# jonathanking/protein-transformer

Measured on AMD Instinct MI355X. Metric: train-step residues/sec (enc-only d512, drmsd loss), higher is better.
Workload: dtype f32 (GEMM and attention operands scaled by powers of two and split into 2 f16 terms [activation x weight products, weight-gradient products whose operands come with a uniform scale, attention with head size 64 / 32] or exactly into 3 bf16 terms [the other weight-gradient products; everything when to; 1 GPU; enc-only d_model=512 n_layers=6 n_head=8 d_ff=2048, -l drmsd, sgd lr 1e-4 wd 0.01 clip 1, dropout 0.1, 32 proteins x L=512 per GPU (BASELINE.json configs[3]); global_batch=32, seq_len=512, parallelism=dp1

## Files before the change

### include/ptamd.h

```cpp
#ifndef PTAMD_H
#define PTAMD_H

#include <stddef.h>
#include <stdint.h>

#ifdef __cplusplus
extern "C" {
#endif

#define PTAMD_OK 0
#define PTAMD_ERR_BAD_SHAPE (-1)
#define PTAMD_ERR_TOO_LONG (-2)
#define PTAMD_ERR_WORKSPACE (-3)
#define PTAMD_ERR_HIP (-4)
#define PTAMD_ERR_ALIGN (-5)

#define PTAMD_ST_BAD_RESIDUE 1
#define PTAMD_ST_TOO_SHORT 2
#define PTAMD_ST_BAD_THETA 4
#define PTAMD_ST_NONFINITE 8

#define PTAMD_PAD_ID 20
#define PTAMD_NUM_ANGLES 12
#define PTAMD_NUM_SLOTS 14
// ... 4 lines not shown

int ptamd_angles_fwd(const float *sincos, float *ang, int64_t n, void *stream);
int ptamd_angles_bwd(const float *sincos, const float *dang, float *dsincos, int64_t n, void *stream);

size_t ptamd_nerf_workspace_bytes(int B, int L);
int ptamd_nerf_place(const float *a, const float *b, const float *c, const float *l, const float *theta,
                     const float *chi, int64_t n, float *d, int32_t *status, void *stream);
int ptamd_pairwise_dist(const float *x, int n, int dim, float *out, void *stream);
int ptamd_nerf_fwd(const float *ang, const int64_t *seq, int B, int L, float *crd, int32_t *status,
                   void *stream);
int ptamd_nerf_bwd(const float *ang, const int64_t *seq, const float *crd, const float *dcrd, int B, int L,
                   float *dang, void *workspace, size_t workspace_bytes, void *stream);

size_t ptamd_drmsd_workspace_bytes(int B, int L);
int ptamd_drmsd_fwd_bwd(const float *pred_crd, const float *true_crd, const int64_t *seq, int B, int L,
                        float *stats, float *dcrd, void *workspace, size_t workspace_bytes, void *stream);
size_t ptamd_drmsd_workspace_bytes_budget(int B, int L, size_t partial_budget_bytes);
int ptamd_drmsd_fwd_bwd_budget(const float *pred_crd, const float *true_crd, const int64_t *seq, int B, int L,
                               float *stats, float *dcrd, void *workspace, size_t workspace_bytes,
                               size_t partial_budget_bytes, void *stream);

int ptamd_kabsch_rmsd(const float *pred_crd, const float *true_crd, const int64_t *seq, int B, int L, float *rmsd,
                      void *stream);

size_t ptamd_mse_angles_workspace_bytes(void);
int ptamd_mse_angles_fwd(const float *pred, const float *truth, int64_t T, float *out, void *workspace,
                         size_t workspace_bytes, void *stream);
int ptamd_mse_angles_bwd(const float *pred, const float *truth, int64_t T, const float *sums, float coef,
                         int accumulate, float *dpred, void *stream);

#define PTAMD_EPI_RELU 1
#define PTAMD_EPI_TANH 2
#define PTAMD_EPI_ACCUM 4
#define PTAMD_EPI_SLABS 16
#define PTAMD_EPI_GATE 8
typedef struct {
  int M, N, K;
  const float *A; int lda; int a_kmajor;
  const float *B; int ldb; int b_kmajor;
  float *C; int ldc;
  const float *bias;
  const float *residual; int ldr;
  int flags;
  float dropout_p; uint64_t seed; uint32_t stream_id;
  int split_k;
  void *workspace; size_t workspace_bytes;
  float *colsum;
  float gate_scale;
  int arith;
  int reserved_cus;
  const uint32_t *a_scale; int a_scale_stride;
  const uint32_t *b_scale; int b_scale_stride;
  const uint64_t *gate_mask;
} ptamd_gemm_args;
size_t ptamd_gate_mask_bytes(int M, int N);
size_t ptamd_gemm_workspace_bytes(int M, int N, int split_k);
int ptamd_gemm(const ptamd_gemm_args *args, void *stream);

#define PTAMD_GEMM_F32 0
#define PTAMD_GEMM_BF16X3 1
#define PTAMD_GEMM_BF16X3_FULL 2
#define PTAMD_GEMM_F16X2 3
#define PTAMD_GEMM_AUTO 4
int ptamd_gemm_products(const ptamd_gemm_args *args);
int ptamd_gemm_group(const ptamd_gemm_args *args, int n, void *stream);

size_t ptamd_hp_bytes(int rows, int K);
int ptamd_hp_padded_rows(int rows);
int ptamd_hp_split(const float *x, int ld, int rows, int K, int transposed, void *planes, float *scale, void *stream);
typedef struct {
  const float *x; int ld, rows, K;
  void *planes; float *scale;
} ptamd_hp_split_job;
int ptamd_hp_split_rows(const ptamd_hp_split_job *jobs_host, int njobs, void *stream);
int ptamd_hp_split_cols(const ptamd_hp_split_job *jobs_host, int njobs, void *stream);
typedef struct {
  int M, N, K;
  const void *A; const float *A_scale;
  const void *B; const float *B_scale;
  float *C; int ldc;
  const float *bias;
  const float *residual; int ldr;
  int flags;
  float dropout_p; uint64_t seed; uint32_t stream_id;
  int split_k;
  void *workspace; size_t workspace_bytes;
  float gate_scale;
  int reserved_cus;
  const uint64_t *gate_mask;
  uint64_t *gate_mask_out;
  void *kv_planes; float *kv_inv; int kv_col0, kv_heads;
} ptamd_gemm_hp_args;
size_t ptamd_gemm_hp_workspace_bytes(int M, int N, int split_k);
int ptamd_gemm_hp(const ptamd_gemm_hp_args *args, void *stream);

typedef struct {
  const float *w; int rows, cols, ld;
  uint32_t *row_scale; uint32_t *col_scale; float *stats;
  int rows_only;
} ptamd_wscale_job;
int ptamd_weight_scales(const ptamd_wscale_job *jobs_host, int njobs, void *stream);
typedef struct {
  const float *ln_gamma_stats; const float *ln_beta_stats;
  const float *w_stats; int w_stat_index;
  const float *bias_stats;
  float sqrt_d, post_scale;
  uint32_t *out_scale; float *out_value;
} ptamd_bound_job;
int ptamd_bound_scales(const ptamd_bound_job *jobs_host, int njobs, void *stream);
typedef struct { uint32_t *dst; int64_t n; uint32_t value; } ptamd_fill_job;
int ptamd_fill_u32(const ptamd_fill_job *jobs_host, int njobs, void *stream);

typedef struct {
  int64_t offset;
  int32_t rows, cols;
  int32_t stats_row0;
  int32_t stats_index;
  int32_t row_scale_index;
  int32_t col_scale_index;
  int32_t colmax_index;
  int32_t colsq_index;
  uint64_t row_planes;
  uint64_t col_planes;
  int32_t ld;
  int32_t rowmax_index;
} ptamd_wprep_seg;
typedef struct {
  int32_t ln_gamma_stats, ln_beta_stats, w_stats, w_stat_index, bias_stats;
  float sqrt_d, post_scale;
  int32_t out_scale, out_value;
} ptamd_wprep_bound;
typedef struct {
  const ptamd_wprep_seg *segs; int32_t nsegs;
  const int32_t *blocks_a; int32_t nblocks_a, nblocks_a_matrices;
  const int64_t *plain; int32_t nplain;
  const int32_t *blocks_b; int32_t nblocks_b;
  const ptamd_wprep_bound *bounds; int32_t nbounds;
  const int32_t *groups; int32_t ngroups;
  const int32_t *colnorm_segs;
  uint32_t *scales; float *values;
  uint32_t *colmax; int32_t ncolmax;
  void *colsq;
  float *stats; int32_t nstats;
  int64_t numel;
// ... 81 lines not shown
```

### protein_transformer_amd/_lib.py

```python
import ctypes as C
import os

import torch

_HERE = os.path.dirname(os.path.abspath(__file__))
_TAG = os.environ.get("PTAMD_LIB_TAG", "")
LIB_PATH = os.path.join(_HERE, "csrc", f"libptamd_{_TAG}.so" if _TAG else "libptamd.so")

OK = 0
ERRORS = {-1: "bad shape", -2: "sequence too long for the NeRF LDS staging", -3: "workspace missing or too small",
          -4: "HIP runtime error", -5: "pointer not 16-byte aligned"}
ST_BAD_RESIDUE, ST_TOO_SHORT, ST_BAD_THETA, ST_NONFINITE = 1, 2, 4, 8

_p, _i, _i64, _f, _sz, _u64, _u32 = C.c_void_p, C.c_int, C.c_int64, C.c_float, C.c_size_t, C.c_uint64, C.c_uint32


class GemmArgs(C.Structure):
    _fields_ = [("M", _i), ("N", _i), ("K", _i),
                ("A", _p), ("lda", _i), ("a_kmajor", _i),
                ("B", _p), ("ldb", _i), ("b_kmajor", _i),
                ("C", _p), ("ldc", _i),
                ("bias", _p),
                ("residual", _p), ("ldr", _i),
                ("flags", _i),
                ("dropout_p", _f), ("seed", _u64), ("stream_id", _u32),
                ("split_k", _i),
                ("workspace", _p), ("workspace_bytes", _sz),
                ("colsum", _p),
                ("gate_scale", _f),
                ("arith", _i),
                ("reserved_cus", _i),
                ("a_scale", _p), ("a_scale_stride", _i),
                ("b_scale", _p), ("b_scale_stride", _i),
                ("gate_mask", _p)]


class WScaleJob(C.Structure):
    _fields_ = [("w", _p), ("rows", _i), ("cols", _i), ("ld", _i), ("row_scale", _p), ("col_scale", _p), ("stats", _p),
                ("rows_only", _i)]


class BoundJob(C.Structure):
    _fields_ = [("ln_gamma_stats", _p), ("ln_beta_stats", _p), ("w_stats", _p), ("w_stat_index", _i), ("bias_stats", _p),
                ("sqrt_d", _f), ("post_scale", _f), ("out_scale", _p), ("out_value", _p)]


class LnReduceJob(C.Structure):
    _fields_ = [("partials", _p), ("D", _i), ("dgamma", _p), ("dbeta", _p)]


class FillJob(C.Structure):
    _fields_ = [("dst", _p), ("n", _i64), ("value", _u32)]


class HpSplitJob(C.Structure):
    _fields_ = [("x", _p), ("ld", _i), ("rows", _i), ("K", _i), ("planes", _p), ("scale", _p)]


class GemmHpArgs(C.Structure):
    _fields_ = [("M", _i), ("N", _i), ("K", _i),
                ("A", _p), ("A_scale", _p),
                ("B", _p), ("B_scale", _p),
                ("C", _p), ("ldc", _i),
                ("bias", _p),
                ("residual", _p), ("ldr", _i),
                ("flags", _i),
                ("dropout_p", _f), ("seed", _u64), ("stream_id", _u32),
                ("split_k", _i),
                ("workspace", _p), ("workspace_bytes", _sz),
                ("gate_scale", _f),
                ("reserved_cus", _i),
                ("gate_mask", _p), ("gate_mask_out", _p),
                ("kv_planes", _p), ("kv_inv", _p), ("kv_col0", _i), ("kv_heads", _i)]


class WprepSeg(C.Structure):
    _fields_ = [("offset", _i64), ("rows", C.c_int32), ("cols", C.c_int32), ("stats_row0", C.c_int32), ("stats_index", C.c_int32),
                ("row_scale_index", C.c_int32), ("col_scale_index", C.c_int32), ("colmax_index", C.c_int32),
                ("colsq_index", C.c_int32), ("row_planes", _u64), ("col_planes", _u64), ("ld", C.c_int32), ("rowmax_index", C.c_int32)]


class WprepBound(C.Structure):
    _fields_ = [("ln_gamma_stats", C.c_int32), ("ln_beta_stats", C.c_int32), ("w_stats", C.c_int32), ("w_stat_index", C.c_int32),
                ("bias_stats", C.c_int32), ("sqrt_d", _f), ("post_scale", _f), ("out_scale", C.c_int32), ("out_value", C.c_int32)]


class WprepPlan(C.Structure):
    _fields_ = [("segs", _p), ("nsegs", C.c_int32),
                ("blocks_a", _p), ("nblocks_a", C.c_int32), ("nblocks_a_matrices", C.c_int32),
                ("plain", _p), ("nplain", C.c_int32),
                ("blocks_b", _p), ("nblocks_b", C.c_int32),
                ("bounds", _p), ("nbounds", C.c_int32),
                ("groups", _p), ("ngroups", C.c_int32),
                ("colnorm_segs", _p),
                ("scales", _p), ("values", _p),
                ("colmax", _p), ("ncolmax", C.c_int32),
                ("colsq", _p),
                ("stats", _p), ("nstats", C.c_int32),
                ("numel", _i64), ("with_planes", C.c_int32)]


SIGNATURES = {
    "ptamd_version": (C.c_char_p, []),
    "ptamd_last_hip_error": (C.c_char_p, []),
    "ptamd_sidechain_atoms": (_i, [_i]),
    "ptamd_angles_fwd": (_i, [_p, _p, _i64, _p]),
    "ptamd_angles_bwd": (_i, [_p, _p, _p, _i64, _p]),
    "ptamd_nerf_workspace_bytes": (_sz, [_i, _i]),
    "ptamd_nerf_place": (_i, [_p, _p, _p, _p, _p, _p, _i64, _p, _p, _p]),
    "ptamd_pairwise_dist": (_i, [_p, _i, _i, _p, _p]),
    "ptamd_nerf_fwd": (_i, [_p, _p, _i, _i, _p, _p, _p]),
    "ptamd_nerf_bwd": (_i, [_p, _p, _p, _p, _i, _i, _p, _p, _sz, _p]),
    "ptamd_drmsd_workspace_bytes": (_sz, [_i, _i]),
    "ptamd_drmsd_fwd_bwd": (_i, [_p, _p, _p, _i, _i, _p, _p, _p, _sz, _p]),
    "ptamd_drmsd_workspace_bytes_budget": (_sz, [_i, _i, _sz]),
    "ptamd_drmsd_fwd_bwd_budget": (_i, [_p, _p, _p, _i, _i, _p, _p, _p, _sz, _sz, _p]),
    "ptamd_kabsch_rmsd": (_i, [_p, _p, _p, _i, _i, _p, _p]),
    "ptamd_mse_angles_workspace_bytes": (_sz, []),
    "ptamd_mse_angles_fwd": (_i, [_p, _p, _i64, _p, _p, _sz, _p]),
    "ptamd_mse_angles_bwd": (_i, [_p, _p, _i64, _p, _f, _i, _p, _p]),
    "ptamd_gemm_workspace_bytes": (_sz, [_i, _i, _i]),
    "ptamd_gate_mask_bytes": (_sz, [_i, _i]),
    "ptamd_gemm": (_i, [C.POINTER(GemmArgs), _p]),
    "ptamd_gemm_products": (_i, [C.POINTER(GemmArgs)]),
    "ptamd_gemm_group": (_i, [C.POINTER(GemmArgs), _i, _p]),
    "ptamd_hp_bytes": (_sz, [_i, _i]),
# ... 113 lines not shown
```

### protein_transformer_amd/csrc/gemm.hip

```cpp
#include <stdlib.h>

#include "gemm_common.h"

namespace ptgemm {
namespace {

template <bool KMAJOR, int BK>
__device__ __forceinline__ void store_stage(float *__restrict__ s, int tid, const float4 (&v)[BK / 8]) {
  constexpr int LPR = BK / 4, LD_R = BK + 4;
#pragma unroll
  for (int i = 0; i < BK / 8; ++i) {
    if (!KMAJOR) {
      const int row = tid / LPR + (NT / LPR) * i, k = 4 * (tid % LPR);
      *reinterpret_cast<float4 *>(s + row * LD_R + k) = v[i];
    } else {
      const int k = (tid >> 5) + 8 * i, row = 4 * (tid & 31);
      *reinterpret_cast<float4 *>(s + k * LD_C + row) = v[i];
    }
  }
}
template <bool KMAJOR, int BK>
__device__ __forceinline__ void read_frag(const float *__restrict__ s, int r, int lh, int m, float (&f)[4]) {
  constexpr int LD_R = BK + 4;
  if (!KMAJOR) {
// ... 329 lines not shown
  const size_t a_bytes = (size_t)(a->a_kmajor ? a->K : a->M) * a->lda * sizeof(float);
  const size_t b_bytes = (size_t)(a->b_kmajor ? a->K : a->N) * a->ldb * sizeof(float);
  if (mode == PTAMD_GEMM_F16X2 && a->K < 32) mode = PTAMD_GEMM_BF16X3;
  if (a->K < 16 || a_bytes >= ((size_t)1 << 32) || b_bytes >= ((size_t)1 << 32)) mode = PTAMD_GEMM_F32;
  return mode;
}
}

int ptamd_gemm_products(const ptamd_gemm_args *a) {
  if (!a || a->M <= 0 || a->N <= 0 || a->K <= 0 || !valid_arith(a->arith)) return PTAMD_ERR_BAD_SHAPE;
  const int mode = resolve_mode(a);
  return mode == PTAMD_GEMM_F32 ? 1 : mode == PTAMD_GEMM_F16X2 ? 3 : mode == PTAMD_GEMM_BF16X3_FULL ? 9 : 6;
}

namespace {
int build_params(const ptamd_gemm_args *a, GemmParams &p, int &splits, int &mode, float *&user_c) {
  if (!a || a->M <= 0 || a->N <= 0 || a->K <= 0 || !valid_arith(a->arith)) return PTAMD_ERR_BAD_SHAPE;
  if ((a->lda & 3) || (a->ldb & 3)) return PTAMD_ERR_BAD_SHAPE;
  if ((!a->a_kmajor || !a->b_kmajor) && (a->K & 3)) return PTAMD_ERR_BAD_SHAPE;
  if (a->a_kmajor && (a->M & 3)) return PTAMD_ERR_BAD_SHAPE;
  if (a->b_kmajor && (a->N & 3)) return PTAMD_ERR_BAD_SHAPE;
  if (!pt_aligned16(a->A) || !pt_aligned16(a->B)) return PTAMD_ERR_ALIGN;
  if (a->dropout_p < 0.f || a->dropout_p >= 1.f) return PTAMD_ERR_BAD_SHAPE;
  splits = a->split_k > 1 ? a->split_k : 1;
  constexpr int BK = 32;
  const int kblocks = (a->K + BK - 1) / BK;
  if (splits > kblocks) splits = kblocks;
  p.M = a->M; p.N = a->N; p.K = a->K;
  p.A = a->A; p.lda = a->lda; p.B = a->B; p.ldb = a->ldb; p.C = a->C; p.ldc = a->ldc;
  p.bias = a->bias; p.residual = a->residual; p.ldr = a->ldr; p.flags = a->flags & ~PTAMD_EPI_SLABS;
  if ((a->flags & PTAMD_EPI_SLABS) && (a->bias || a->residual || a->colsum || a->gate_mask || a->dropout_p != 0.f ||
                                      (a->flags & (PTAMD_EPI_RELU | PTAMD_EPI_TANH | PTAMD_EPI_ACCUM | PTAMD_EPI_GATE))))
    return PTAMD_ERR_BAD_SHAPE;
  p.dropout_p = a->dropout_p; p.seed = a->seed; p.stream_id = a->stream_id; p.gate_scale = a->gate_scale;
  p.reserved_cus = a->reserved_cus;
  p.k_per_split = ((kblocks + splits - 1) / splits) * BK;
  splits = (a->K + p.k_per_split - 1) / p.k_per_split;
  p.splits = splits;
  p.vec_epilogue = !(a->N & 3) && !(a->ldc & 3) && pt_aligned16(a->C) &&
                   (!a->residual || (!(a->ldr & 3) && pt_aligned16(a->residual))) &&
                   (splits == 1 || pt_aligned16(a->workspace));
  p.slab = 0;
  p.colsum = a->colsum;
  p.colsum_share = 1;
  {
    const int tiles_n = (a->N + BN - 1) / BN;
    while (p.colsum_share * 2 <= tiles_n && p.colsum_share < 16) p.colsum_share *= 2;
  }
  if (a->colsum && !a->a_kmajor) return PTAMD_ERR_BAD_SHAPE;
  if ((a->flags & PTAMD_EPI_GATE) && (a->residual == nullptr) == (a->gate_mask == nullptr)) return PTAMD_ERR_BAD_SHAPE;
  if (a->gate_mask && !(a->flags & PTAMD_EPI_GATE)) return PTAMD_ERR_BAD_SHAPE;
  p.gate_mask = a->gate_mask; p.gate_mask_out = nullptr;
  p.mask_rb = (a->M + 31) / 32; p.mask_cb = (a->N + 31) / 32;
  user_c = a->C;
  if (splits > 1) {
    if (!a->workspace || a->workspace_bytes < slab_bytes(a->M, a->N, splits)) return PTAMD_ERR_WORKSPACE;
    p.slab = (size_t)a->M * a->N;
    p.C = static_cast<float *>(a->workspace);
    if (a->colsum) p.colsum = p.C + (size_t)splits * p.slab;
  }
  mode = resolve_mode(a);
  if (a->gate_mask && (mode != PTAMD_GEMM_F16X2 || !p.vec_epilogue || splits > 1 || a->dropout_p != 0.f)) return PTAMD_ERR_BAD_SHAPE;
  p.scale_a = p.scale_b = nullptr;
  p.scale_a_stride = p.scale_b_stride = 1;
  if (mode == PTAMD_GEMM_F16X2) {
    if (a->a_scale && a->a_scale_stride != 0 && a->a_scale_stride != 1) return PTAMD_ERR_BAD_SHAPE;
    if (a->b_scale && a->b_scale_stride != 0 && a->b_scale_stride != 1) return PTAMD_ERR_BAD_SHAPE;
  }
  return PTAMD_OK;
}
}

size_t ptamd_gate_mask_bytes(int M, int N) {
  if (M <= 0 || N <= 0) return 0;
  return (size_t)((M + 31) / 32) * ((N + 31) / 32) * 16 * sizeof(uint64_t);
}

int ptamd_gemm(const ptamd_gemm_args *a, void *stream) {
  GemmParams p;
  int splits, mode;
  float *user_c;
  if (const int rc = build_params(a, p, splits, mode, user_c)) return rc;
  hipStream_t st = (hipStream_t)stream;
  if (mode == PTAMD_GEMM_F16X2) {
    uint32_t *sa = nullptr, *sb = nullptr;
    if (!a->a_scale || !a->b_scale) {
      if (!a->workspace || !pt_aligned16(a->workspace) || a->workspace_bytes < ptamd_gemm_workspace_bytes(a->M, a->N, splits))
        return PTAMD_ERR_WORKSPACE;
      uint32_t *ws = reinterpret_cast<uint32_t *>(static_cast<char *>(a->workspace) + slab_bytes(a->M, a->N, splits));
      if (!a->a_scale) sa = ws;
      if (!a->b_scale) sb = ws + round4(a->M);
      if (const int rs = launch_row_scales(p, a->a_kmajor != 0, a->b_kmajor != 0, sa, sb, st)) return rs;
    }
    p.scale_a = a->a_scale ? a->a_scale : sa;
    p.scale_b = a->b_scale ? a->b_scale : sb;
    p.scale_a_stride = a->a_scale ? a->a_scale_stride : 1;
    p.scale_b_stride = a->b_scale ? a->b_scale_stride : 1;
  }
  const int products = mode == PTAMD_GEMM_BF16X3_FULL ? 9 : mode == PTAMD_GEMM_F16X2 ? 3 : 6;
  const int rc = mode == PTAMD_GEMM_F32 ? launch_f32(p, a->a_kmajor != 0, a->b_kmajor != 0, splits, st)
                                        : launch_split(p, a->a_kmajor != 0, a->b_kmajor != 0, splits, products, st);
  if (rc || splits == 1 || (a->flags & PTAMD_EPI_SLABS)) return rc;
  const float *slabs = p.C;
  p.C = user_c;
  const float *cs_slabs = a->colsum ? slabs + (size_t)splits * p.slab : nullptr;
  return launch_splitk_reduce(p, slabs, splits, cs_slabs, a->colsum, st);
}

int ptamd_gemm_group(const ptamd_gemm_args *args, int n, void *stream) {
  if (!args || n <= 0 || n > MAX_GROUP) return PTAMD_ERR_BAD_SHAPE;
  GemmGroup g;
  ReduceGroup r;
  g.n = r.n = n;
  int items = 0, blocks = 0;
// ... 40 lines not shown
```

### protein_transformer_amd/csrc/gemm_common.h

```cpp
#pragma once
#include "common.h"

namespace ptgemm {

typedef float f32x16 __attribute__((ext_vector_type(16)));
typedef float f32x4 __attribute__((ext_vector_type(4)));

constexpr int BM = 128, BN = 128, NT = 256;
constexpr int LD_C = 132;

struct GemmParams {
  int M, N, K;
  const float *A;
  int lda;
  const float *B;
  int ldb;
  float *C;
  int ldc;
  const float *bias;
  const float *residual;
  int ldr;
  int flags;
  float dropout_p;
  uint64_t seed;
  uint32_t stream_id;
  int k_per_split;
  int splits;
  size_t slab;
  int vec_epilogue;
  float *colsum;
  int colsum_share;
  float gate_scale;
  const uint32_t *scale_a, *scale_b;
  int scale_a_stride, scale_b_stride;
  int reserved_cus;
  const uint64_t *gate_mask;
  uint64_t *gate_mask_out;
  int mask_rb, mask_cb;
};
__device__ __forceinline__ uint32_t load_gate_masks(const GemmParams &p, int rb, int cb, int lane) {
  const int rbu = __builtin_amdgcn_readfirstlane(rb), cbu = __builtin_amdgcn_readfirstlane(cb);
  const bool in = rbu < p.mask_rb && cbu < p.mask_cb;
  const uint32_t *src = reinterpret_cast<const uint32_t *>(p.gate_mask + ((size_t)(in ? cbu : 0) * p.mask_rb + (in ? rbu : 0)) * 16);
  return src[lane & 31];
}
__device__ __forceinline__ bool gate_keep(uint32_t masks, int r) {
  const uint32_t lo = (uint32_t)__builtin_amdgcn_readlane((int)masks, 2 * r), hi = (uint32_t)__builtin_amdgcn_readlane((int)masks, 2 * r + 1);
  return __builtin_amdgcn_inverse_ballot_w64(((uint64_t)hi << 32) | lo);
}

template <bool KMAJOR, int BK>
__device__ __forceinline__ void load_stage(const float *__restrict__ src, int ld, int rows, int r0, int kend, int k0,
                                           int tid, float4 (&v)[BK / 8]) {
  constexpr int LPR = BK / 4;
#pragma unroll
  for (int i = 0; i < BK / 8; ++i) {
    if (!KMAJOR) {
      const int row = r0 + tid / LPR + (NT / LPR) * i, k = k0 + 4 * (tid % LPR);
      v[i] = (row < rows && k < kend) ? *reinterpret_cast<const float4 *>(src + (size_t)row * ld + k)
                                      : make_float4(0.f, 0.f, 0.f, 0.f);
    } else {
      const int k = k0 + (tid >> 5) + 8 * i, row = r0 + 4 * (tid & 31);
      v[i] = (k < kend && row < rows) ? *reinterpret_cast<const float4 *>(src + (size_t)k * ld + row)
                                      : make_float4(0.f, 0.f, 0.f, 0.f);
    }
  }
}
__device__ __forceinline__ float epilogue_value(float v, int row, int col, const GemmParams &p, uint32_t thr,
                                                float keep_scale) {
  if (p.bias) v += p.bias[col];
  if (p.flags & PTAMD_EPI_RELU) v = fmaxf(v, 0.f);
  if (p.dropout_p > 0.f) v = drop_keep(p.seed, p.stream_id, row, col, p.N, thr >> 16) ? v * keep_scale : 0.f;
  if (p.residual) {
    const float r = p.residual[(size_t)row * p.ldr + col];
    v = (p.flags & PTAMD_EPI_GATE) ? (r > 0.f ? v * p.gate_scale : 0.f) : v + r;
  }
  if (p.flags & PTAMD_EPI_TANH) v = tanhf(v);
  return v;
}


constexpr int EPI_PLAIN = 0, EPI_NODROP = 1, EPI_FULL = 2;
template <int TI, bool VEC = true, int EPI = EPI_FULL, bool MASK_GATE = false>
__device__ __forceinline__ void tile_epilogue_vec(const GemmParams &p, const f32x16 (&acc)[TI][2], float *C, int ldc,
                                                  bool partial, int row0, int col0, int lane, uint32_t thr,
                                                  float keep_scale, float *scratch) {
  const int l31 = lane & 31, lh = lane >> 5;
  uint32_t keep[TI];
#pragma unroll
  for (int i = 0; i < TI; ++i) keep[i] = 0xffffffffu;
  if (EPI == EPI_FULL && !partial && p.dropout_p > 0.f) {
// ... 172 lines not shown
```

### protein_transformer_amd/csrc/gemm_hp.hip

```cpp
#include <stdlib.h>

#include "gemm_common.h"
#include "hp_format.h"
#include "kv_format.h"
#include "split_bf16.h"

extern "C" __device__ int pt_llvm_amdgcn_writelane(int value, int lane, int old) __asm("llvm.amdgcn.writelane");

namespace pthp {
namespace {

using ptgemm::GemmParams;
using ptgemm::f32x16;
using ptsplit::f16x8;

constexpr int HBN = 128;

struct HpParams {
  GemmParams g;
  const char *a_planes, *b_planes;
  const float *a_scale, *b_scale;
  int kb16;
  int a_rb_last, b_rb_last;
  char *kv_planes;
  float *kv_inv;
  int kv_col0, kv_heads, kv_nt;
};

typedef __attribute__((address_space(1))) const void *gptr_t;
typedef __attribute__((address_space(3))) void *lptr_t;
__device__ __forceinline__ void dma16(const char *g, char *l) {
  __builtin_amdgcn_global_load_lds((gptr_t)g, (lptr_t)l, 16, 0, 0);
}

struct Item {
  int bm0, bn0, z, kbeg, kend;
};
struct Cursor {
  int w, k0;
  Item it;
};

template <int WM_, int TI_, int KB_, bool ILV_>
struct HpGeom {
  static constexpr int WM = WM_, TI = TI_, KB = KB_;
  static constexpr bool ILV = ILV_;
  static constexpr int NW = 2 * WM, THREADS = 64 * NW, TILE_M = 32 * TI * WM, BK = 16 * KB;
  static constexpr int A_BLOCKS = TILE_M / 32, B_BLOCKS = HBN / 32;
  static constexpr int RB_BYTES = KB * 2048;
  static constexpr int A_STAGE = A_BLOCKS * RB_BYTES, STAGE_BYTES = (A_BLOCKS + B_BLOCKS) * RB_BYTES;
  static constexpr int PIECES = STAGE_BYTES / 1024, PER_WAVE = PIECES / NW;
  static constexpr int SCRATCH_BYTES = NW * 2048 * 4;
  static constexpr size_t LDS = (size_t)2 * STAGE_BYTES + SCRATCH_BYTES;
  static constexpr int WG_PER_CU = LDS <= 80 * 1024 ? 2 : 1;
  static_assert(PIECES % NW == 0, "pieces must divide evenly over the wavefronts");
  static_assert(LDS <= 160 * 1024, "LDS budget of a CU");
};

template <typename G, int EPI>
__global__ __launch_bounds__(G::THREADS, G::WG_PER_CU * G::NW / 4) void gemm_hp_kernel(const HpParams p) {
  constexpr int TI = G::TI, KB = G::KB, BK = G::BK;
  extern __shared__ __attribute__((aligned(16))) char smem[];
  float *const scratch = reinterpret_cast<float *>(smem + 2 * G::STAGE_BYTES);
  const int tid = threadIdx.x, lane = tid & 63;
  const int wave = __builtin_amdgcn_readfirstlane(tid >> 6);
  const int wm = wave >> 1, wn = wave & 1;
  const ptgemm::WorkRange work(p.g, G::TILE_M, HBN);
  if (work.begin >= work.end) return;
  const int Kp = p.kb16 * 16;
  auto item_at = [&](int logical) __attribute__((always_inline)) {
    Item it;
    work.decode(logical, it.bm0, it.bn0, it.z);
    it.kbeg = it.z * p.g.k_per_split;
    it.kend = min(Kp, it.kbeg + p.g.k_per_split);
    return it;
  };
  auto advance = [&](Cursor &c) __attribute__((always_inline)) {
    if (c.k0 + BK < c.it.kend) {
      c.k0 += BK;
// ... 53 lines not shown
        __builtin_amdgcn_sched_barrier(0);
        if (more_loads) {
#pragma unroll
          for (int u = 0; u < n; ++u)
            if (piece + u < G::PER_WAVE) issue_piece(ld, buf ^ 1, piece + u);
        }
        piece += n;
        __builtin_amdgcn_sched_barrier(0);
      }
    };
    constexpr int SLOTS = 3 * KB, PER_SLOT = (G::PER_WAVE + SLOTS - 1) / SLOTS;
    f16x8 fa[TI][2], fb[2][2];
#pragma unroll
    for (int kb = 0; kb < KB; ++kb) {
#pragma unroll
      for (int t = 0; t < 2; ++t) {
#pragma unroll
        for (int i = 0; i < TI; ++i) fa[i][t] = *reinterpret_cast<const f16x8 *>(sa + i * G::RB_BYTES + (kb * 2 + t) * 1024);
#pragma unroll
        for (int j = 0; j < 2; ++j) fb[j][t] = *reinterpret_cast<const f16x8 *>(sb + j * G::RB_BYTES + (kb * 2 + t) * 1024);
      }
#pragma unroll
      for (int i = 0; i < TI; ++i)
#pragma unroll
        for (int j = 0; j < 2; ++j) acc[i][j] = __builtin_amdgcn_mfma_f32_32x32x16_f16(fa[i][1], fb[j][0], acc[i][j], 0, 0, 0);
      dma_slot(PER_SLOT);
#pragma unroll
      for (int i = 0; i < TI; ++i)
#pragma unroll
        for (int j = 0; j < 2; ++j) acc[i][j] = __builtin_amdgcn_mfma_f32_32x32x16_f16(fa[i][0], fb[j][1], acc[i][j], 0, 0, 0);
      dma_slot(PER_SLOT);
#pragma unroll
      for (int i = 0; i < TI; ++i)
#pragma unroll
        for (int j = 0; j < 2; ++j) acc[i][j] = __builtin_amdgcn_mfma_f32_32x32x16_f16(fa[i][0], fb[j][0], acc[i][j], 0, 0, 0);
      dma_slot(PER_SLOT);
    }
    if (more_loads) more_loads = advance(ld);
    if (cc.k0 + BK >= cc.it.kend) {
      float *C = p.g.C + (partial ? (size_t)cc.it.z * p.g.slab : 0);
      const int ldc = partial ? p.g.N : p.g.ldc;
      const int row0 = cc.it.bm0 + wm * 32 * TI, col0 = cc.it.bn0 + wn * 64;
      {
        const int l31 = lane & 31, lh = lane >> 5;
        float ib[2];
#pragma unroll
        for (int j = 0; j < 2; ++j) ib[j] = inverse_of_scale(p.b_scale[min(col0 + j * 32 + l31, p.g.N - 1)]);
#pragma unroll
        for (int i = 0; i < TI; ++i)
#pragma unroll
          for (int g = 0; g < 4; ++g)
#pragma unroll
            for (int e = 0; e < 4; ++e) {
              const float ia = inverse_of_scale(p.a_scale[min(row0 + i * 32 + 8 * g + 4 * lh + e, p.g.M - 1)]);
#pragma unroll
              for (int j = 0; j < 2; ++j) acc[i][j][g * 4 + e] = acc[i][j][g * 4 + e] * ia * ib[j];
            }
      }
      if (p.g.vec_epilogue)
        ptgemm::tile_epilogue_vec<TI, true, EPI>(p.g, acc, C, ldc, partial, row0, col0, lane, thr, keep_scale, scratch + wave * 2048);
      else
        ptgemm::tile_epilogue_vec<TI, false, EPI>(p.g, acc, C, ldc, partial, row0, col0, lane, thr, keep_scale, scratch + wave * 2048);
      zero_acc();
    }
    if (!advance(cc)) break;
    buf ^= 1;
  }
}

template <typename G, int EPI>
int launch_hp_g(const HpParams &p, int splits, hipStream_t st) {
  const int work = ((p.g.M + G::TILE_M - 1) / G::TILE_M) * ((p.g.N + HBN - 1) / HBN) * splits;
  auto kern = gemm_hp_kernel<G, EPI>;
  PT_HIP_TRY(hipFuncSetAttribute(reinterpret_cast<const void *>(kern), hipFuncAttributeMaxDynamicSharedMemorySize, (int)G::LDS));
  const int slots = ptgemm::persistent_grid(p.g.reserved_cus) * G::WG_PER_CU;
  hipLaunchKernelGGL(kern, dim3(work < slots ? work : slots), dim3(G::THREADS), G::LDS, st, p);
  return pt_check_launch();
}

typedef HpGeom<4, 2, 2, true> Geom;

template <int EPI, bool KVP = false>
int launch_hp3(const HpParams &p, int splits, hipStream_t st);
template <int EPI>
int launch_hp(const HpParams &p, int splits, hipStream_t st) {
  if (p.g.vec_epilogue) return launch_hp3<EPI == ptgemm::EPI_NODROP ? ptgemm::EPI_FULL : EPI>(p, splits, st);
  if (p.g.gate_mask_out) return PTAMD_ERR_BAD_SHAPE;
  return launch_hp_g<Geom, EPI>(p, splits, st);
}

struct Hp3 {
  static constexpr int WM = 4, NW = 2 * WM, THREADS = 64 * NW, TILE_M = 64 * WM, BK = 32, NSTAGE = 3;
  static constexpr int A_BLOCKS = 2 * WM, B_BLOCKS = 4, PER_WAVE = (A_BLOCKS + B_BLOCKS) * 4 / NW;
  static constexpr int RB_BYTES = 4096, A_STAGE = A_BLOCKS * RB_BYTES, STAGE_BYTES = (A_BLOCKS + B_BLOCKS) * RB_BYTES;
  static constexpr int SCRATCH_BYTES = NW * 2048;
  static constexpr size_t LDS = (size_t)NSTAGE * STAGE_BYTES + SCRATCH_BYTES;
  static_assert(LDS <= 160 * 1024, "the LDS of a CU");
};

__device__ __forceinline__ void kv_split8(const float4 &a, const float4 &b, float s, uint4 &hi, uint4 &lo) {
  uint2 h0, l0, h1, l1;
  ptsplit::split_quad_f16(a.x, a.y, a.z, a.w, s, s, s, s, h0, l0);
  ptsplit::split_quad_f16(b.x, b.y, b.z, b.w, s, s, s, s, h1, l1);
  hi = make_uint4(h0.x, h0.y, h1.x, h1.y);
  lo = make_uint4(l0.x, l0.y, l1.x, l1.y);
}
__device__ __forceinline__ uint32_t half_umax(uint32_t v) {
  v = max(v, (uint32_t)__builtin_amdgcn_update_dpp(0, (int)v, 0xB1, 0xF, 0xF, true));
  v = max(v, (uint32_t)__builtin_amdgcn_update_dpp(0, (int)v, 0x4E, 0xF, 0xF, true));
  v = max(v, (uint32_t)__builtin_amdgcn_update_dpp(0, (int)v, 0x141, 0xF, 0xF, true));
  v = max(v, (uint32_t)__builtin_amdgcn_update_dpp(0, (int)v, 0x140, 0xF, 0xF, true));
  v = max(v, (uint32_t)__shfl_xor((int)v, 16, 64));
  return v;
}

template <int EPI, bool KVP = false>
__device__ __forceinline__ void hp3_epilogue(const GemmParams &p, const f32x16 (&acc)[2][2], float *C, int ldc, bool partial,
                                             int row0, int col0, int lane, uint32_t thr, float keep_scale, float *scratch,
                                             const HpParams *hp = nullptr) {
  using ptgemm::EPI_FULL;
  using ptgemm::EPI_PLAIN;
  typedef float f32x4 __attribute__((ext_vector_type(4)));
  const int l31 = lane & 31, lh = lane >> 5;
  uint32_t keep[2] = {0xffffffffu, 0xffffffffu};
  if (EPI == EPI_FULL && !partial && p.dropout_p > 0.f) {
    keep[0] = keep[1] = 0u;
#pragma unroll 4
    for (int idx = 0; idx < 8; ++idx) {
      const int i = idx >> 2, j = (idx >> 1) & 1, gp = idx & 1;
      const int row = row0 + i * 32 + 16 * gp + 4 * lh, col = col0 + j * 32 + l31;
      const uint4 rnd = pt_rand4(p.seed, drop_call_index(row, col, p.N), p.stream_id);
      const uint32_t t16 = thr >> 16;
      uint32_t bits = 0;
#pragma unroll
      for (int f = 0; f < 8; ++f)
        bits |= (drop_field_value(rnd, f) >= t16 ? 1u : 0u) << (j * 16 + (2 * gp + (f >> 2)) * 4 + (f & 3));
      keep[0] |= i == 0 ? bits : 0u;
      keep[1] |= i == 1 ? bits : 0u;
    }
  }
#pragma unroll
  for (int i = 0; i < 2; ++i) {
    __builtin_amdgcn_sched_barrier(0);
    f32x4 pre4[8];
    const bool want_res = EPI != EPI_PLAIN && !partial && p.residual != nullptr;
    const bool want_old = EPI != EPI_PLAIN && !partial && (p.flags & PTAMD_EPI_ACCUM) && !want_res;
#pragma unroll
    for (int t = 0; t < 8; ++t) {
      const int f = lane + 64 * t, rr = f >> 4, c4 = (f & 15) * 4;
      const int row = min(row0 + i * 32 + rr, p.M - 1), col = min(col0 + c4, p.N - 4);
      const float *src = want_res ? p.residual + (size_t)row * p.ldr + col : C + (size_t)row * ldc + col;
      pre4[t] = (f32x4){0.f, 0.f, 0.f, 0.f};
      if (want_res || want_old) pre4[t] = *reinterpret_cast<const f32x4 *>(src);
    }
    float bias[2];
#pragma unroll
    for (int j = 0; j < 2; ++j) {
      const int col = col0 + j * 32 + l31;
      bias[j] = (EPI != EPI_PLAIN && !partial && p.bias && col < p.N) ? p.bias[col] : 0.f;
    }
    int mask_lo[2] = {0, 0}, mask_hi[2] = {0, 0};
    const bool gated = EPI != EPI_PLAIN && !partial && p.gate_mask != nullptr;
    uint32_t gmk[2] = {0u, 0u};
    if (gated) {
      gmk[0] = ptgemm::load_gate_masks(p, (row0 >> 5) + i, col0 >> 5, lane);
      gmk[1] = ptgemm::load_gate_masks(p, (row0 >> 5) + i, (col0 >> 5) + 1, lane);
    }
#pragma unroll
    for (int g = 0; g < 4; ++g) {
#pragma unroll
      for (int j = 0; j < 2; ++j)
#pragma unroll
        for (int e = 0; e < 4; ++e) {
          float v = acc[i][j][g * 4 + e];
          if (EPI != EPI_PLAIN && !partial) {
            v += bias[j];
            if (p.flags & PTAMD_EPI_RELU) v = fmaxf(v, 0.f);
            if (EPI == EPI_FULL && p.dropout_p > 0.f) v = (keep[i] >> (j * 16 + g * 4 + e)) & 1u ? v * keep_scale : 0.f;
            if (gated) v = ptgemm::gate_keep(gmk[j], g * 4 + e) ? v * p.gate_scale : 0.f;
            if (p.gate_mask_out) {
              const uint64_t m = __builtin_amdgcn_ballot_w64(v > 0.f);
              mask_lo[j] = pt_llvm_amdgcn_writelane((int)(uint32_t)m, g * 4 + e, mask_lo[j]);
              mask_hi[j] = pt_llvm_amdgcn_writelane((int)(uint32_t)(m >> 32), g * 4 + e, mask_hi[j]);
            }
          }
          scratch[(4 * lh + e) * 64 + j * 32 + l31] = v;
        }
      if (KVP && col0 >= hp->kv_col0) {
        const int rr = lane >> 3, ch = lane & 7;
        const float4 a = *reinterpret_cast<const float4 *>(scratch + rr * 64 + ch * 8);
        const float4 b = *reinterpret_cast<const float4 *>(scratch + rr * 64 + ch * 8 + 4);
        const uint32_t am = half_umax(max(max(max(__float_as_uint(a.x) & 0x7fffffffu, __float_as_uint(a.y) & 0x7fffffffu),
                                              max(__float_as_uint(a.z) & 0x7fffffffu, __float_as_uint(a.w) & 0x7fffffffu)),
                                          max(max(__float_as_uint(b.x) & 0x7fffffffu, __float_as_uint(b.y) & 0x7fffffffu),
                                              max(__float_as_uint(b.z) & 0x7fffffffu, __float_as_uint(b.w) & 0x7fffffffu))));
        const uint32_t sbits = pt_row_scale_bits(am);
        uint4 hi, lo;
        kv_split8(a, b, __uint_as_float(sbits), hi, lo);
        const int hc = (col0 - hp->kv_col0) >> 6;
        const int gt = (row0 >> 5) + i, r = 8 * g + rr;
        if (row0 + i * 32 < p.M) {
          char *tile = hp->kv_planes + ((size_t)hc * hp->kv_nt + gt) * ptkv::TILE_BYTES;
          char *dst = tile + r * ptkv::ROW_BYTES + ptkv::chunk_pos(r, ch) * 16;
          *reinterpret_cast<uint4 *>(dst) = hi;
          *reinterpret_cast<uint4 *>(dst + ptkv::PLANE_BYTES) = lo;
          if ((lane & 31) == 0)
            hp->kv_inv[((size_t)hc * hp->kv_nt + gt) * 8 + ptkv::group_slot(2 * g + lh)] = __uint_as_float((254u << 23) - sbits);
        }
        continue;
      }
#pragma unroll
      for (int u = 0; u < 2; ++u) {
        const int f = lane + 64 * u, rr = f >> 4, c4 = (f & 15) * 4;
        const int row = row0 + i * 32 + 8 * g + rr, col = col0 + c4;
        float4 v = *reinterpret_cast<const float4 *>(scratch + rr * 64 + c4);
#ifdef PT_ABLATE_NOSTORE
        if (row < p.M && col < p.N && p.M < 0) {
#else
        if (row < p.M && col < p.N) {
#endif
          if (EPI != EPI_PLAIN && !partial) {
            const f32x4 r4 = pre4[2 * g + u];
            if (p.residual) {
              if (p.flags & PTAMD_EPI_GATE) {
                v.x = r4.x > 0.f ? v.x * p.gate_scale : 0.f; v.y = r4.y > 0.f ? v.y * p.gate_scale : 0.f;
                v.z = r4.z > 0.f ? v.z * p.gate_scale : 0.f; v.w = r4.w > 0.f ? v.w * p.gate_scale : 0.f;
              } else {
                v.x += r4.x; v.y += r4.y; v.z += r4.z; v.w += r4.w;
              }
            }
            if (p.flags & PTAMD_EPI_TANH) { v.x = tanhf(v.x); v.y = tanhf(v.y); v.z = tanhf(v.z); v.w = tanhf(v.w); }
            if (p.flags & PTAMD_EPI_ACCUM) {
              const f32x4 o4 = want_old ? r4 : *reinterpret_cast<const f32x4 *>(C + (size_t)row * ldc + col);
              v.x += o4.x; v.y += o4.y; v.z += o4.z; v.w += o4.w;
            }
          }
          *reinterpret_cast<float4 *>(C + (size_t)row * ldc + col) = v;
        }
      }
    }
    if (EPI != EPI_PLAIN && !partial && p.gate_mask_out) {
      const int rb = __builtin_amdgcn_readfirstlane((row0 >> 5) + i);
#pragma unroll
      for (int j = 0; j < 2; ++j) {
        const int cb = __builtin_amdgcn_readfirstlane((col0 >> 5) + j);
        if (lane < 16 && rb < p.mask_rb && cb < p.mask_cb)
          p.gate_mask_out[((size_t)cb * p.mask_rb + rb) * 16 + lane] = ((uint64_t)(uint32_t)mask_hi[j] << 32) | (uint32_t)mask_lo[j];
      }
    }
  }
}

#define PT_DS_READ_B128(dst, addr, off) asm volatile("ds_read_b128 %0, %1 offset:%2" : "=v"(dst) : "v"(addr), "n"(off))

template <int EPI, bool KVP = false>
__global__ __launch_bounds__(Hp3::THREADS, 2) void gemm_hp3_kernel(const HpParams p) {
  using G = Hp3;
  extern __shared__ __attribute__((aligned(16))) char smem[];
  float *const scratch = reinterpret_cast<float *>(smem + G::NSTAGE * G::STAGE_BYTES);
  const int tid = threadIdx.x, lane = tid & 63;
  const int wave = __builtin_amdgcn_readfirstlane(tid >> 6);
  const int wm = wave >> 1, wn = wave & 1;
  const ptgemm::WorkRange work(p.g, G::TILE_M, HBN);
  if (work.begin >= work.end) return;
  const int Kp = p.kb16 * 16;
  auto item_at = [&](int logical) __attribute__((always_inline)) {
    Item it;
    work.decode(logical, it.bm0, it.bn0, it.z);
    it.kbeg = it.z * p.g.k_per_split;
    it.kend = min(Kp, it.kbeg + p.g.k_per_split);
    return it;
  };
  auto advance = [&](Cursor &c) __attribute__((always_inline)) {
    if (c.k0 + G::BK < c.it.kend) {
      c.k0 += G::BK;
      return true;
    }
    if (c.w + 1 < work.end) {
      c.it = item_at(++c.w);
      c.k0 = c.it.kbeg;
      return true;
    }
    return false;
  };
  const int rb_in_tile = wave >> 2, rest_bytes = (wave & 3) * 1024;
  const char *const a_base = p.a_planes + rest_bytes + lane * 16, *const b_base = p.b_planes + rest_bytes + lane * 16;
  const int64_t row_bytes = (int64_t)p.kb16 * 2048;
  auto issue_piece = [&](const Cursor &c, int buf, int i) __attribute__((always_inline)) {
    const int q = wave + G::NW * i;
    const bool is_b = i >= 4;
    const int rb = is_b ? min((c.it.bn0 >> 5) + 2 * (i - 4) + rb_in_tile, p.b_rb_last)
                        : min((c.it.bm0 >> 5) + 2 * i + rb_in_tile, p.a_rb_last);
    const char *g = (is_b ? b_base : a_base) + (int64_t)rb * row_bytes + (int64_t)(c.k0 >> 4) * 2048;
    dma16(g, smem + buf * G::STAGE_BYTES + q * 1024);
  };

  f32x16 acc[2][2];
  auto zero_acc = [&]() __attribute__((always_inline)) {
#pragma unroll
    for (int i = 0; i < 2; ++i)
#pragma unroll
      for (int j = 0; j < 2; ++j)
#pragma unroll
        for (int r = 0; r < 16; ++r) acc[i][j][r] = 0.f;
  };
  zero_acc();
  const uint32_t thr = dropout_threshold(p.g.dropout_p);
  const float keep_scale = 1.f / (1.f - p.g.dropout_p);
// ... 33 lines not shown
    PT_DS_READ_B128(fa[0][1][0], va, 4096);
    PT_DS_READ_B128(fa[0][1][1], va, 4096 + 1024);
    PT_DS_READ_B128(fb[0][1][0], vb, 4096);
    PT_DS_READ_B128(fb[0][1][1], vb, 4096 + 1024);
    PT_DS_READ_B128(fa[1][0][0], va, 2048);
    PT_DS_READ_B128(fa[1][0][1], va, 2048 + 1024);
    PT_DS_READ_B128(fb[1][0][0], vb, 2048);
    PT_DS_READ_B128(fb[1][0][1], vb, 2048 + 1024);
    PT_DS_READ_B128(fa[1][1][0], va, 4096 + 2048);
    PT_DS_READ_B128(fa[1][1][1], va, 4096 + 2048 + 1024);
    PT_DS_READ_B128(fb[1][1][0], vb, 4096 + 2048);
    PT_DS_READ_B128(fb[1][1][1], vb, 4096 + 2048 + 1024);
    const bool issue = more_loads;
#pragma unroll
    for (int kb = 0; kb < 2; ++kb) {
      if (kb == 0) asm volatile("s_waitcnt lgkmcnt(8)" ::: "memory");
      else asm volatile("s_waitcnt lgkmcnt(0)" ::: "memory");
      __builtin_amdgcn_sched_barrier(0);
#pragma unroll
      for (int pr = 0; pr < 3; ++pr) {
        const int ta = pr == 0 ? 1 : 0, tb = pr == 1 ? 1 : 0;
#pragma unroll
        for (int i = 0; i < 2; ++i)
#pragma unroll
          for (int j = 0; j < 2; ++j)
            acc[i][j] = __builtin_amdgcn_mfma_f32_32x32x16_f16(fa[kb][i][ta], fb[kb][j][tb], acc[i][j], 0, 0, 0);
        __builtin_amdgcn_sched_barrier(0);
        if (issue) issue_piece(ld, nbuf, kb * 3 + pr);
        __builtin_amdgcn_sched_barrier(0);
      }
    }
    if (issue) {
      more_loads = advance(ld);
      ++ahead;
    }
    --ahead;
    if (cc.k0 + G::BK >= cc.it.kend) {
      asm volatile("s_waitcnt vmcnt(0)" ::: "memory");
      landed = ahead;
      float *C = p.g.C + (partial ? (size_t)cc.it.z * p.g.slab : 0);
      const int ldc = partial ? p.g.N : p.g.ldc;
      const int row0 = cc.it.bm0 + wm * 64, col0 = cc.it.bn0 + wn * 64;
      {
        const int l31 = lane & 31, lh = lane >> 5;
        float ib[2];
#pragma unroll
        for (int j = 0; j < 2; ++j) ib[j] = inverse_of_scale(p.b_scale[min(col0 + j * 32 + l31, p.g.N - 1)]);
#pragma unroll
        for (int i = 0; i < 2; ++i)
#pragma unroll
          for (int g = 0; g < 4; ++g)
#pragma unroll
            for (int e = 0; e < 4; ++e) {
              const float ia = inverse_of_scale(p.a_scale[min(row0 + i * 32 + 8 * g + 4 * lh + e, p.g.M - 1)]);
#pragma unroll
              for (int j = 0; j < 2; ++j) acc[i][j][g * 4 + e] = acc[i][j][g * 4 + e] * ia * ib[j];
            }
      }
      hp3_epilogue<EPI, KVP>(p.g, acc, C, ldc, partial, row0, col0, lane, thr, keep_scale, scratch + wave * 512, &p);
      zero_acc();
    }
    if (!advance(cc)) break;
    buf = buf == G::NSTAGE - 1 ? 0 : buf + 1;
  }
}

template <int EPI, bool KVP>
int launch_hp3(const HpParams &p, int splits, hipStream_t st) {
  const int work = ((p.g.M + Hp3::TILE_M - 1) / Hp3::TILE_M) * ((p.g.N + HBN - 1) / HBN) * splits;
  auto kern = gemm_hp3_kernel<EPI, KVP>;
  PT_HIP_TRY(hipFuncSetAttribute(reinterpret_cast<const void *>(kern), hipFuncAttributeMaxDynamicSharedMemorySize, (int)Hp3::LDS));
  const int slots = ptgemm::persistent_grid(p.g.reserved_cus);
  hipLaunchKernelGGL(kern, dim3(work < slots ? work : slots), dim3(Hp3::THREADS), Hp3::LDS, st, p);
  return pt_check_launch();
}

__global__ __launch_bounds__(256) void hp_rowscale_kernel(const float *__restrict__ x, int ld, int rows, int K, int rows_p,
                                                          float *__restrict__ scale) {
  const int r = blockIdx.x * 4 + (threadIdx.x >> 6), lane = threadIdx.x & 63;
  if (r >= rows_p) return;
  if (r >= rows) {
    if (lane == 0) scale[r] = 1.f;
    return;
  }
  const float *p = x + (size_t)r * ld;
  float m = 0.f;
  for (int k = lane * 4; k < K; k += 256) {
    const float4 v = *reinterpret_cast<const float4 *>(p + k);
    m = fmaxf(fmaxf(m, fmaxf(fabsf(v.x), fabsf(v.y))), fmaxf(fabsf(v.z), fabsf(v.w)));
  }
  m = wave_max(m);
  if (lane == 0) scale[r] = __uint_as_float(scale_bits_of(__float_as_uint(m)));
}
__global__ __launch_bounds__(256) void hp_colmax_kernel(const float *__restrict__ x, int ld, int rows, int K,
                                                        uint32_t *__restrict__ amax) {
  const int r = blockIdx.x * 256 + threadIdx.x;
  if (r >= rows) return;
  const int k0 = blockIdx.y * 64, k1 = min(K, k0 + 64);
  float m = 0.f;
  for (int k = k0; k < k1; ++k) m = fmaxf(m, fabsf(x[(size_t)k * ld + r]));
  atomicMax(amax + r, __float_as_uint(m));
}
__global__ __launch_bounds__(256) void hp_amax_to_scale_kernel(uint32_t *__restrict__ amax_scale, int rows, int rows_p) {
  const int r = blockIdx.x * 256 + threadIdx.x;
  if (r < rows_p) amax_scale[r] = r < rows ? scale_bits_of(amax_scale[r]) : 0x3f800000u;
}
template <bool TRANSPOSED, bool SCALE_IS_AMAX>
__global__ __launch_bounds__(256) void hp_write_kernel(const float *__restrict__ x, int ld, int rows, int K, int kb16v,
                                                       const float *__restrict__ scale, char *__restrict__ planes,
                                                       int64_t nchunks) {
  const int64_t id = (int64_t)blockIdx.x * 256 + threadIdx.x;
  if (id >= nchunks) return;
  const int c = (int)(id & 63);
  const int64_t blk = id >> 6;
  const int kb = (int)(blk % kb16v), rb = (int)(blk / kb16v);
  int r, h;
  chunk_coords(c, r, h);
  const int row = rb * 32 + r, k0 = kb * 16 + h * 8;
  float v[8];
#pragma unroll
  for (int e = 0; e < 8; ++e) v[e] = 0.f;
  float s = 1.f;
  if (row < rows) {
// ... 141 lines not shown
                       rows, rows_p);
  }
  return pt_check_launch();
}

int ptamd_hp_split_rows(const ptamd_hp_split_job *jobs, int njobs, void *stream) {
  if (!jobs || njobs <= 0 || njobs > MAX_SPLIT_JOBS) return PTAMD_ERR_BAD_SHAPE;
  SplitJobs j;
  int blocks = 0, kmax = 0;
  for (int i = 0; i < njobs; ++i) {
    const ptamd_hp_split_job &q = jobs[i];
    if (!q.x || !q.planes || !q.scale || q.rows <= 0 || q.K <= 0 || (q.K & 3) || (q.ld & 3) || q.K > 2048) return PTAMD_ERR_BAD_SHAPE;
    if (!pt_aligned16(q.x) || !pt_aligned16(q.planes)) return PTAMD_ERR_ALIGN;
    j.x[i] = q.x; j.planes[i] = static_cast<char *>(q.planes); j.scale[i] = q.scale;
    j.ld[i] = q.ld; j.rows[i] = q.rows; j.K[i] = q.K;
    j.first_block[i] = blocks;
    blocks += round_up(q.rows, 32) / 4;
    kmax = q.K > kmax ? q.K : kmax;
  }
  for (int i = njobs; i <= MAX_SPLIT_JOBS; ++i) j.first_block[i] = blocks;
  j.njobs = njobs;
  hipStream_t st = (hipStream_t)stream;
  if (kmax <= 256) hipLaunchKernelGGL(hp_split_rows_kernel<1>, dim3(blocks), dim3(256), 0, st, j);
  else if (kmax <= 512) hipLaunchKernelGGL(hp_split_rows_kernel<2>, dim3(blocks), dim3(256), 0, st, j);
  else if (kmax <= 1024) hipLaunchKernelGGL(hp_split_rows_kernel<4>, dim3(blocks), dim3(256), 0, st, j);
  else hipLaunchKernelGGL(hp_split_rows_kernel<8>, dim3(blocks), dim3(256), 0, st, j);
  return pt_check_launch();
}

int ptamd_hp_split_cols(const ptamd_hp_split_job *jobs, int njobs, void *stream) {
  if (!jobs || njobs <= 0 || njobs > MAX_SPLIT_JOBS) return PTAMD_ERR_BAD_SHAPE;
  SplitColsJobs j;
  int blocks = 0;
  for (int i = 0; i < njobs; ++i) {
    const ptamd_hp_split_job &q = jobs[i];
    if (!q.x || !q.planes || !q.scale || q.rows <= 0 || q.K <= 0 || q.ld < q.rows) return PTAMD_ERR_BAD_SHAPE;
    if (!pt_aligned16(q.planes)) return PTAMD_ERR_ALIGN;
    j.x[i] = q.x; j.planes[i] = static_cast<char *>(q.planes); j.scale[i] = q.scale;
    j.ld[i] = q.ld; j.rows[i] = q.rows; j.K[i] = q.K;
    j.first_block[i] = blocks;
    const int64_t nchunks = (int64_t)(round_up(q.rows, 32) / 32) * kb16(q.K) * 64;
    blocks += (int)((nchunks + 255) / 256);
  }
  for (int i = njobs; i <= MAX_SPLIT_JOBS; ++i) j.first_block[i] = blocks;
  j.njobs = njobs;
  hipLaunchKernelGGL(hp_split_cols_kernel, dim3(blocks), dim3(256), 0, (hipStream_t)stream, j);
  return pt_check_launch();
}

size_t ptamd_gemm_hp_workspace_bytes(int M, int N, int split_k) { return (M <= 0 || N <= 0) ? 0 : slab_bytes(M, N, split_k); }

int ptamd_gemm_hp(const ptamd_gemm_hp_args *a, void *stream) {
  if (!a || a->M <= 0 || a->N <= 0 || a->K <= 0) return PTAMD_ERR_BAD_SHAPE;
  if (!a->A || !a->B || !a->A_scale || !a->B_scale || !a->C) return PTAMD_ERR_BAD_SHAPE;
  if (!pt_aligned16(a->A) || !pt_aligned16(a->B)) return PTAMD_ERR_ALIGN;
  if (a->dropout_p < 0.f || a->dropout_p >= 1.f) return PTAMD_ERR_BAD_SHAPE;
  if ((a->flags & PTAMD_EPI_GATE) && (a->residual == nullptr) == (a->gate_mask == nullptr)) return PTAMD_ERR_BAD_SHAPE;
  if (a->gate_mask && !(a->flags & PTAMD_EPI_GATE)) return PTAMD_ERR_BAD_SHAPE;
  HpParams p;
  GemmParams &g = p.g;
  g.M = a->M; g.N = a->N; g.K = a->K;
  g.A = nullptr; g.lda = 0; g.B = nullptr; g.ldb = 0; g.C = a->C; g.ldc = a->ldc;
  g.bias = a->bias; g.residual = a->residual; g.ldr = a->ldr; g.flags = a->flags;
  g.dropout_p = a->dropout_p; g.seed = a->seed; g.stream_id = a->stream_id; g.gate_scale = a->gate_scale;
  g.reserved_cus = a->reserved_cus;
  g.colsum = nullptr; g.colsum_share = 1; g.scale_a = g.scale_b = nullptr; g.scale_a_stride = g.scale_b_stride = 1;
  g.gate_mask = a->gate_mask; g.gate_mask_out = a->gate_mask_out;
  g.mask_rb = (a->M + 31) / 32; g.mask_cb = (a->N + 31) / 32;
  constexpr int HBK = 32;
  const int Kp = round_up(a->K, 32), stages = Kp / HBK;
  int splits = a->split_k > 1 ? a->split_k : 1;
  if (splits > stages) splits = stages;
  g.k_per_split = ((stages + splits - 1) / splits) * HBK;
  splits = (Kp + g.k_per_split - 1) / g.k_per_split;
  g.splits = splits;
  g.vec_epilogue = !(a->N & 3) && !(a->ldc & 3) && pt_aligned16(a->C) &&
                   (!a->residual || (!(a->ldr & 3) && pt_aligned16(a->residual))) && (splits == 1 || pt_aligned16(a->workspace));
  g.slab = 0;
  float *user_c = a->C;
  if (splits > 1) {
    if (!a->workspace || a->workspace_bytes < slab_bytes(a->M, a->N, splits)) return PTAMD_ERR_WORKSPACE;
    g.slab = (size_t)a->M * a->N;
    g.C = static_cast<float *>(a->workspace);
  }
  p.a_planes = static_cast<const char *>(a->A);
  p.b_planes = static_cast<const char *>(a->B);
  p.a_scale = a->A_scale;
  p.b_scale = a->B_scale;
  p.kb16 = Kp / 16;
  p.a_rb_last = (round_up(a->M, 32) / 32) - 1;
  p.b_rb_last = (round_up(a->N, 32) / 32) - 1;
  p.kv_planes = static_cast<char *>(a->kv_planes);
  p.kv_inv = a->kv_inv;
  p.kv_col0 = a->kv_col0;
  p.kv_heads = a->kv_heads;
  p.kv_nt = a->M / 32;
  hipStream_t st = (hipStream_t)stream;
  if (a->kv_planes) {
    if (!a->kv_inv || a->kv_heads <= 0 || (a->M & 31) || (a->kv_col0 & 63) || a->kv_col0 < 0 ||
        a->N != a->kv_col0 + 2 * a->kv_heads * 64 || !g.vec_epilogue || splits > 1 || a->residual || a->gate_mask ||
        a->gate_mask_out || a->dropout_p != 0.f || a->flags != 0)
      return PTAMD_ERR_BAD_SHAPE;
    if (!pt_aligned16(a->kv_planes)) return PTAMD_ERR_ALIGN;
    return launch_hp3<ptgemm::EPI_FULL, true>(p, 1, st);
  }
  const bool plain = !a->bias && !a->residual && !a->gate_mask && !a->gate_mask_out &&
                     !(a->flags & (PTAMD_EPI_RELU | PTAMD_EPI_TANH | PTAMD_EPI_ACCUM)) && a->dropout_p == 0.f;
  if ((a->gate_mask || a->gate_mask_out) && (!g.vec_epilogue || splits > 1)) return PTAMD_ERR_BAD_SHAPE;
  int rc;
  if (plain || splits > 1) rc = launch_hp<ptgemm::EPI_PLAIN>(p, splits, st);
  else if (a->dropout_p == 0.f) rc = launch_hp<ptgemm::EPI_NODROP>(p, splits, st);
  else rc = launch_hp<ptgemm::EPI_FULL>(p, splits, st);
  if (rc || splits == 1) return rc;
  const float *slabs = g.C;
  g.C = user_c;
  return ptgemm::launch_splitk_reduce(g, slabs, splits, nullptr, nullptr, st);
}

}
```

### protein_transformer_amd/csrc/gemm_split_kernel.h

```cpp
#pragma once
#include <type_traits>

#include <stdlib.h>

#include "gemm_common.h"
#include "split_bf16.h"

namespace ptgemm {
namespace {

using namespace ptsplit;

constexpr int TBN = 128;
constexpr int NTHREADS = 512, NPRODUCER = 256;
constexpr int KR_PAD = 32;
constexpr int SCRATCH_FLOATS = 4 * 2048;
constexpr int COLSUM_AREAS = 3;
constexpr int COLSUM_FLOATS = COLSUM_AREAS * 4 * 256;
constexpr int cmax(int a, int b) { return a > b ? a : b; }

template <int NPROD, int TI = 4>
struct Geo {
  static constexpr int TBM = 64 * TI;
  static constexpr bool F16 = NPROD == 3;
// ... 57 lines not shown
#pragma unroll
  for (int i = 0; i < NV; ++i) {
    const int kl = KMAJOR ? pt / LPK + (NPRODUCER / LPK) * i : 4 * (pt % G::QK);
    uint2 t1, t2, t3;
    split_pair(v[i].x, v[i].y, t1.x, t2.x, t3.x);
    split_pair(v[i].z, v[i].w, t1.y, t2.y, t3.y);
    const int off = KMAJOR ? kl * LD_KR + 4 * (pt % LPK)
                           : G::rk_offset(pt / G::QK + (NPRODUCER / G::QK) * i, kl);
    *reinterpret_cast<uint2 *>(s + off) = t1;
    *reinterpret_cast<uint2 *>(s + PLANE + off) = t2;
    *reinterpret_cast<uint2 *>(s + 2 * PLANE + off) = t3;
  }
}

constexpr int MAX_NV = 8;
template <typename G, bool KMAJOR, int ROWS>
__device__ __forceinline__ void scale_offsets(int rows, int r0, int pt, uint32_t (&soff)[MAX_NV], int stride = 1) {
  constexpr int LPK = ROWS / 4, NV = G::template nv<ROWS>();
#pragma unroll
  for (int i = 0; i < MAX_NV; ++i) {
    if (!KMAJOR) soff[i] = (uint32_t)min(r0 + pt / G::QK + (NPRODUCER / G::QK) * (i < NV ? i : 0), rows - 1) * 4u * (uint32_t)stride;
    else soff[i] = (uint32_t)min(r0 + 4 * (pt % LPK), rows - 4) * 4u * (uint32_t)stride;
  }
}
template <typename G, bool KMAJOR, int ROWS>
__device__ __forceinline__ void load_scales(const uint32_t *__restrict__ scale, const uint32_t (&soff)[MAX_NV], float (&sc)[MAX_NV]) {
  const char *base = reinterpret_cast<const char *>(scale);
  constexpr int NV = G::template nv<ROWS>();
  if (!KMAJOR) {
#pragma unroll
    for (int i = 0; i < NV; ++i) sc[i] = *reinterpret_cast<const float *>(base + soff[i]);
  } else {
    const float4 v = *reinterpret_cast<const float4 *>(base + soff[0]);
    sc[0] = v.x; sc[1] = v.y; sc[2] = v.z; sc[3] = v.w;
  }
}
template <typename G, bool KMAJOR, int ROWS>
__device__ __forceinline__ void store_split_f16_one(unsigned short *__restrict__ s, int pt, const float4 &v, const float (&sc)[MAX_NV], int i) {
  constexpr int LPK = ROWS / 4, PLANE = G::template plane<ROWS>(), LD_KR = ROWS + KR_PAD;
  const int kl = KMAJOR ? pt / LPK + (NPRODUCER / LPK) * i : 4 * (pt % G::QK);
  uint2 t1, t2;
  split_quad_f16(v.x, v.y, v.z, v.w, KMAJOR ? sc[0] : sc[i], KMAJOR ? sc[1] : sc[i], KMAJOR ? sc[2] : sc[i], KMAJOR ? sc[3] : sc[i], t1, t2);
  const int off = KMAJOR ? kl * LD_KR + 4 * (pt % LPK) : G::rk_offset(pt / G::QK + (NPRODUCER / G::QK) * i, kl);
  *reinterpret_cast<uint2 *>(s + off) = t1;
  *reinterpret_cast<uint2 *>(s + PLANE + off) = t2;
}
template <typename G, bool KMAJOR, int ROWS>
__device__ __forceinline__ void store_split_f16(unsigned short *__restrict__ s, int pt, const float4 (&v)[G::template nv<ROWS>()],
                                                const float (&sc)[MAX_NV]) {
  constexpr int NV = G::template nv<ROWS>();
#pragma unroll
  for (int i = 0; i < NV; ++i) store_split_f16_one<G, KMAJOR, ROWS>(s, pt, v[i], sc, i);
}
__device__ __forceinline__ uint32_t row_scale_bits(uint32_t amax) { return min(268u - (amax >> 23), 254u) << 23; }
__device__ __forceinline__ float inverse_scale(uint32_t scale_bits) { return __uint_as_float((254u << 23) - scale_bits); }

template <typename G, bool KMAJOR, int ROWS>
__device__ __forceinline__ bf16x8 read_frag(const unsigned short *__restrict__ s, int r0, int lane, int t, int ks) {
  constexpr int PLANE = G::template plane<ROWS>(), LD_KR = ROWS + KR_PAD;
  if (!KMAJOR) {
    return *reinterpret_cast<const bf16x8 *>(s + t * PLANE + G::rk_offset(r0 + (lane & 31), 16 * ks + 8 * (lane >> 5)));
  } else {
    const int q16 = lane & 15;
    const unsigned short *q = s + t * PLANE + (16 * ks + 8 * (lane >> 5) + (q16 >> 2)) * LD_KR + r0 + (lane & 16) + 4 * (q16 & 3);
    const s16x4 lo = __builtin_amdgcn_ds_read_tr16_b64_v4i16((lds_s16x4 *)q);
    const s16x4 hi = __builtin_amdgcn_ds_read_tr16_b64_v4i16((lds_s16x4 *)(q + 4 * LD_KR));
    const s16x8 both = __builtin_shufflevector(lo, hi, 0, 1, 2, 3, 4, 5, 6, 7);
    return __builtin_bit_cast(bf16x8, both);
  }
}

struct Item {
  int bm0, bn0, z, kbeg, kend, pj;
};

struct Cursor {
  int w, k0;
  Item it;
  bool end;
};

template <bool GROUPED>
struct KernelArg {
  typedef GemmParams type;
};
template <>
struct KernelArg<true> {
  typedef GemmGroup type;
};
template <bool A_KMAJOR, bool B_KMAJOR, int NPROD, int EPI, int TI = 4, bool GROUPED = false>
__global__ __launch_bounds__(NTHREADS, 1) __attribute__((amdgpu_waves_per_eu(2, 2))) void gemm_bf16x3_mfma_kernel(
    const typename KernelArg<GROUPED>::type arg) {
  extern __shared__ __attribute__((aligned(16))) unsigned short smem[];
  using G = Geo<NPROD, TI>;
  constexpr int TBM = G::TBM;
  static_assert(TI == 4 || !A_KMAJOR, "the fused bias gradient of k-major A assumes 256-row tiles");
  constexpr int SBK = G::SBK, NSETS = G::NSETS, STAGE = G::STAGE, PLANE_A = G::PLANE_A, NVA = G::NVA, NVB = G::NVB;
  float *const scratch = reinterpret_cast<float *>(smem + 2 * STAGE);
  float *const cs_area = scratch + SCRATCH_FLOATS;

  constexpr bool F16 = NPROD == 3;
  const int tid = threadIdx.x, lane = tid & 63, wave = tid >> 6;
  auto P = [&](int j) __attribute__((always_inline)) -> const GemmParams & {
    if constexpr (GROUPED) return arg.p[j];
    else return arg;
  };
  typename std::conditional<GROUPED, GroupRange, WorkRange>::type work(arg, TBM, TBN);
  if (work.begin >= work.end) return;
  auto item_at = [&](int logical) __attribute__((always_inline)) {
    Item it;
    if constexpr (GROUPED) work.decode(arg, logical, it.pj, it.bm0, it.bn0, it.z);
    else {
      work.decode(logical, it.bm0, it.bn0, it.z);
      it.pj = 0;
    }
    it.kbeg = it.z * P(it.pj).k_per_split;
    it.kend = min(P(it.pj).K, it.kbeg + P(it.pj).k_per_split);
    return it;
  };
  auto advance = [&](Cursor &c) __attribute__((always_inline)) {
    if (c.k0 + SBK < c.it.kend) {
      c.k0 += SBK;
    } else if (c.w + 1 < work.end) {
      c.it = item_at(++c.w);
      c.k0 = c.it.kbeg;
    } else {
      c.end = true;
    }
  };
  int total_stages = 0;
  for (int w = work.begin; w < work.end; ++w) {
    const Item it = item_at(w);
    total_stages += (it.kend - it.kbeg + SBK - 1) / SBK;
  }
  const int padded_stages = (total_stages + NSETS - 1) / NSETS * NSETS;
  const bool partial = P(0).slab != 0;
  const bool has_colsum = A_KMAJOR && P(0).colsum != nullptr;
  auto cs_share_of = [&](const Item &it) __attribute__((always_inline)) { return partial ? P(it.pj).colsum_share : 1; };
  auto colsum_first = [&](const Item &it) __attribute__((always_inline)) { return (it.bn0 / TBN) & (cs_share_of(it) - 1); };
  auto colsum_on = [&](const Item &it) __attribute__((always_inline)) {
    return has_colsum && (partial ? it.bn0 / TBN < cs_share_of(it) : it.bn0 == 0);
  };

  if (wave >= 4) {
    const int pt = tid - NPRODUCER;
    float4 csum = make_float4(0.f, 0.f, 0.f, 0.f);
    float cs_w[NVA];
#pragma unroll
    for (int i = 0; i < NVA; ++i) cs_w[i] = 0.f;
    int cs_parity = 0;
    auto colsum_weights = [&](const Item &it) __attribute__((always_inline)) {
      const bool on = colsum_on(it);
      const int first = colsum_first(it), cs_share = cs_share_of(it);
#pragma unroll
      for (int i = 0; i < NVA; ++i) cs_w[i] = (on && ((pt / 64 + 4 * i) & (cs_share - 1)) == first) ? 1.f : 0.f;
    };

    Cursor ld = {work.begin, 0, item_at(work.begin), false};
    ld.k0 = ld.it.kbeg;
    Cursor st = ld;
    colsum_weights(st.it);
    uint32_t voa[NVA], vob[NVB];
    const float *opA = P(ld.it.pj).A, *opB = P(ld.it.pj).B;
    int op_lda = P(ld.it.pj).lda, op_ldb = P(ld.it.pj).ldb;
    item_offsets<G, A_KMAJOR, TBM>(op_lda, P(ld.it.pj).M, ld.it.bm0, pt, voa);
    item_offsets<G, B_KMAJOR, TBN>(op_ldb, P(ld.it.pj).N, ld.it.bn0, pt, vob);
    float4 ra[NSETS][NVA], rb[NSETS][NVB];
    float rsa[NSETS][MAX_NV], rsb[NSETS][MAX_NV];
    uint32_t soa[MAX_NV], sob[MAX_NV];
    if (F16) {
      scale_offsets<G, A_KMAJOR, TBM>(P(ld.it.pj).M, ld.it.bm0, pt, soa, P(ld.it.pj).scale_a_stride);
      scale_offsets<G, B_KMAJOR, TBN>(P(ld.it.pj).N, ld.it.bn0, pt, sob, P(ld.it.pj).scale_b_stride);
    }
    int rskip[NSETS];
    auto fetch_tail = [&](float (&sa_)[MAX_NV], float (&sb_)[MAX_NV]) __attribute__((always_inline)) {
      if (F16 && ld.k0 - ld.it.kbeg < NSETS * SBK) {
        load_scales<G, A_KMAJOR, TBM>(P(ld.it.pj).scale_a, soa, sa_);
        load_scales<G, B_KMAJOR, TBN>(P(ld.it.pj).scale_b, sob, sb_);
      }
      const int w_before = ld.w;
      advance(ld);
      if (ld.w != w_before) {
        if (GROUPED) {
          opA = P(ld.it.pj).A; opB = P(ld.it.pj).B;
          op_lda = P(ld.it.pj).lda; op_ldb = P(ld.it.pj).ldb;
        }
        item_offsets<G, A_KMAJOR, TBM>(op_lda, P(ld.it.pj).M, ld.it.bm0, pt, voa);
        item_offsets<G, B_KMAJOR, TBN>(op_ldb, P(ld.it.pj).N, ld.it.bn0, pt, vob);
        if (F16) {
          scale_offsets<G, A_KMAJOR, TBM>(P(ld.it.pj).M, ld.it.bm0, pt, soa, P(ld.it.pj).scale_a_stride);
          scale_offsets<G, B_KMAJOR, TBN>(P(ld.it.pj).N, ld.it.bn0, pt, sob, P(ld.it.pj).scale_b_stride);
        }
      }
    };
    auto fetch = [&](float4 (&a)[NVA], float4 (&b)[NVB], int &kskip, float (&sa_)[MAX_NV], float (&sb_)[MAX_NV]) __attribute__((always_inline)) {
      const int klim = ld.it.kend - ld.k0;
      const int ks = klim >= SBK ? ld.k0 : ld.it.kend - SBK;
      kskip = ld.k0 - ks;
      load_raw(opA + (A_KMAJOR ? (size_t)ks * op_lda : (size_t)ks), voa, a);
      load_raw(opB + (B_KMAJOR ? (size_t)ks * op_ldb : (size_t)ks), vob, b);
      fetch_tail(sa_, sb_);
    };
    auto produce = [&](float4 (&a)[NVA], float4 (&b)[NVB], int &kskip, float (&sa_)[MAX_NV], float (&sb_)[MAX_NV], int buf) __attribute__((always_inline)) {
      unsigned short *sa = smem + buf * STAGE, *sb = sa + G::NPLANES * PLANE_A;
      mask_tail<G, A_KMAJOR, TBM>(pt, a, kskip);
      mask_tail<G, B_KMAJOR, TBN>(pt, b, kskip);
      if (has_colsum) {
#pragma unroll
        for (int i = 0; i < NVA; ++i) {
          csum.x = fmaf(cs_w[i], a[i].x, csum.x); asm volatile("" : "+v"(csum.x));
          csum.y = fmaf(cs_w[i], a[i].y, csum.y); asm volatile("" : "+v"(csum.y));
          csum.z = fmaf(cs_w[i], a[i].z, csum.z); asm volatile("" : "+v"(csum.z));
          csum.w = fmaf(cs_w[i], a[i].w, csum.w); asm volatile("" : "+v"(csum.w));
        }
      }
      if (F16) {
        const int klim = ld.it.kend - ld.k0;
        const int ks_next = klim >= SBK ? ld.k0 : ld.it.kend - SBK;
        const float *na = opA + (A_KMAJOR ? (size_t)ks_next * op_lda : (size_t)ks_next);
        const float *nb = opB + (B_KMAJOR ? (size_t)ks_next * op_ldb : (size_t)ks_next);
        constexpr int GRP = 2;
#pragma unroll
        for (int i0 = 0; i0 < NVA; i0 += GRP) {
#pragma unroll
          for (int i = i0; i < i0 + GRP && i < NVA; ++i) store_split_f16_one<G, A_KMAJOR, TBM>(sa, pt, a[i], sa_, i);
          __builtin_amdgcn_sched_barrier(0);
#pragma unroll
          for (int i = i0; i < i0 + GRP && i < NVA; ++i)
            a[i] = *reinterpret_cast<const float4 *>(reinterpret_cast<const char *>(na) + voa[i]);
          __builtin_amdgcn_sched_barrier(0);
        }
#pragma unroll
        for (int i0 = 0; i0 < NVB; i0 += GRP) {
#pragma unroll
          for (int i = i0; i < i0 + GRP && i < NVB; ++i) store_split_f16_one<G, B_KMAJOR, TBN>(sb, pt, b[i], sb_, i);
          __builtin_amdgcn_sched_barrier(0);
#pragma unroll
          for (int i = i0; i < i0 + GRP && i < NVB; ++i)
            b[i] = *reinterpret_cast<const float4 *>(reinterpret_cast<const char *>(nb) + vob[i]);
          __builtin_amdgcn_sched_barrier(0);
        }
        kskip = ld.k0 - ks_next;
      } else {
        store_split<G, A_KMAJOR, TBM>(sa, pt, a);
        store_split<G, B_KMAJOR, TBN>(sb, pt, b);
      }
      if (has_colsum && !st.end && st.k0 + SBK >= st.it.kend) {
        if (colsum_on(st.it)) {
          reinterpret_cast<float4 *>(cs_area + cs_parity * 4 * TBM)[pt] = csum;
          cs_parity = cs_parity == COLSUM_AREAS - 1 ? 0 : cs_parity + 1;
        }
        csum = make_float4(0.f, 0.f, 0.f, 0.f);
      }
      {
        const int w_before = st.w;
        const bool was_end = st.end;
        advance(st);
        if (st.w != w_before) colsum_weights(st.it);
        if (st.end && !was_end) {
#pragma unroll
          for (int i = 0; i < NVA; ++i) cs_w[i] = 0.f;
        }
      }
      __builtin_amdgcn_sched_barrier(0);
      if (F16) fetch_tail(sa_, sb_);
      else fetch(a, b, kskip, sa_, sb_);
    };
#pragma unroll
    for (int u = 0; u < NSETS; ++u) {
      fetch(ra[u], rb[u], rskip[u], rsa[u], rsb[u]);
      __builtin_amdgcn_sched_barrier(0);
    }
    produce(ra[0], rb[0], rskip[0], rsa[0], rsb[0], 0);
    __syncthreads();
    for (int g = 0; g < padded_stages; g += NSETS) {
#pragma unroll
      for (int u = 1; u <= NSETS; ++u) {
        produce(ra[u % NSETS], rb[u % NSETS], rskip[u % NSETS], rsa[u % NSETS], rsb[u % NSETS], u & 1);
        __syncthreads();
      }
    }
  } else {
    const int wm = wave >> 1, wn = wave & 1;
    f32x16 acc[TI][2];
    auto zero_acc = [&]() __attribute__((always_inline)) {
#pragma unroll
      for (int i = 0; i < TI; ++i)
#pragma unroll
// ... 155 lines not shown
```

### protein_transformer_amd/csrc/wprep.hip

```cpp
#include "common.h"
#include "hp_format.h"
#include "optim_update.h"
#include "split_bf16.h"

namespace {

constexpr int RB = 32, WAVES = 4, RW = RB / WAVES, MAXV = 2;
constexpr int PLAIN_F4 = 4096;

struct OptArgs {
  int kind;
  int zero_g;
  float *g;
  float *m, *v;
  const float *sqnorm;
  float max_norm, lr, wd, beta1, beta2, eps, step_size, inv_sqrt_bc2;
};

using ptopt::clip_coef;
using ptopt::sgd_update;
__device__ __forceinline__ float adam_update(float p, float g, float &m, float &v, float coef, const OptArgs &o) {
  return ptopt::adam_update(p, g, m, v, coef, o.wd, o.beta1, o.beta2, o.eps, o.step_size, o.inv_sqrt_bc2);
}
template <int KIND>
// ... 181 lines not shown
      atomicMax(pl.colmax + sg.colmax_index + c, __float_as_uint(mx));
    }
  }
  if (want_sq) {
    double (*s_d)[64 * 4 * MAXV] = reinterpret_cast<double (*)[64 * 4 * MAXV]>(&s_col[0][0]);
    double *dst = pl.colsq + sg.colsq_index + (int64_t)blk.y * cols;
    __syncthreads();
#pragma unroll
    for (int i = 0; i < MAXV; ++i) {
      const int c = (i * 64 + lane) * 4;
      if (i < nv && c < cols) {
        s_d[wave][c] = cs[i][0]; s_d[wave][c + 1] = cs[i][1]; s_d[wave][c + 2] = cs[i][2]; s_d[wave][c + 3] = cs[i][3];
      }
    }
    __syncthreads();
    for (int c = tid; c < cols; c += 64 * WAVES) dst[c] = ((s_d[0][c] + s_d[1][c]) + s_d[2][c]) + s_d[3][c];
  }
}

struct PlanB {
  const ptamd_wprep_seg *segs;
  const int4 *blocks;
  const ptamd_wprep_bound *bounds;
  const int4 *groups;
  const int *colnorm_segs;
  uint32_t *scales;
  float *values;
  const uint32_t *colmax;
  uint32_t *colmax_next;
  const double *colsq;
  float *stats;
  float *stats_next;
  int nstats, with_planes;
};

__global__ __launch_bounds__(256) void wprep_cols_kernel(const float *__restrict__ w, const PlanB pl) {
  const int4 blk = pl.blocks[blockIdx.x];
  const int tid = threadIdx.x;
  if (blk.x == 0) {
    const ptamd_wprep_seg sg = pl.segs[blk.y];
    for (int c = blk.z * 2048 + tid; c < min(sg.cols, (blk.z + 1) * 2048); c += 256) {
      pl.scales[sg.col_scale_index + c] = pt_row_scale_bits(pl.colmax[sg.colmax_index + c]);
      pl.colmax_next[sg.colmax_index + c] = 0u;
    }
    return;
  }
  if (blk.x == 3) {
    const ptamd_wprep_seg sg = pl.segs[blk.y];
    const int r = blk.z * 256 + tid;
    if (r < sg.rows) {
      pl.scales[sg.row_scale_index + r] = pt_row_scale_bits(pl.colmax[sg.rowmax_index + r]);
      pl.colmax_next[sg.rowmax_index + r] = 0u;
    }
    return;
  }
  if (blk.x == 1) {
    if (!pl.with_planes) return;
    const ptamd_wprep_seg sg = pl.segs[blk.y];
    const int rows = sg.cols, K = sg.rows, kbv = pthp::kb16(K), ld = sg.ld;
    const int64_t nchunks = (int64_t)(pthp::round_up(rows, 32) / 32) * kbv * 64;
    const int64_t id = (int64_t)blk.z * 256 + tid;
    if (id >= nchunks) return;
    const int c = (int)(id & 63);
    const int64_t b = id >> 6;
    const int kb = (int)(b % kbv), rb = (int)(b / kbv);
    int r, h;
    pthp::chunk_coords(c, r, h);
    const int row = rb * 32 + r, k0 = kb * 16 + h * 8;
    float v[8];
#pragma unroll
    for (int e = 0; e < 8; ++e) v[e] = 0.f;
    float sc = 1.f;
    if (row < rows) {
      sc = __uint_as_float(pt_row_scale_bits(pl.colmax[sg.colmax_index + row]));
      const float *x = w + sg.offset;
#pragma unroll
      for (int e = 0; e < 8; ++e)
        if (k0 + e < K) v[e] = x[(size_t)(k0 + e) * ld + row];
    }
    uint4 hi, lo;
    ptsplit::split_pair_f16(v[0], v[1], sc, sc, hi.x, lo.x);
    ptsplit::split_pair_f16(v[2], v[3], sc, sc, hi.y, lo.y);
    ptsplit::split_pair_f16(v[4], v[5], sc, sc, hi.z, lo.z);
    ptsplit::split_pair_f16(v[6], v[7], sc, sc, hi.w, lo.w);
    char *dst = reinterpret_cast<char *>(sg.col_planes) + pthp::block_offset(rb, kb, 0, kbv) + c * 16;
    *reinterpret_cast<uint4 *>(dst) = hi;
    *reinterpret_cast<uint4 *>(dst + pthp::BLK_BYTES) = lo;
    return;
  }
  const int4 grp = pl.groups[blk.y];
  __shared__ float s_red[4];
  for (int e = 0; e < grp.w; ++e) {
    const ptamd_wprep_seg sg = pl.segs[pl.colnorm_segs[grp.z + e]];
    const int nb = (sg.rows + RB - 1) / RB;
    float nmax = 0.f;
    for (int c = tid; c < sg.cols; c += 256) {
      const double *q = pl.colsq + sg.colsq_index + c;
      double s0 = 0.0, s1 = 0.0, s2 = 0.0, s3 = 0.0;
      int b = 0;
      for (; b + 8 <= nb; b += 8) {
        double t[8];
#pragma unroll
        for (int u = 0; u < 8; ++u) t[u] = q[(int64_t)(b + u) * sg.cols];
        s0 += t[0]; s1 += t[1]; s2 += t[2]; s3 += t[3];
        s0 += t[4]; s1 += t[5]; s2 += t[6]; s3 += t[7];
      }
// ... 101 lines not shown
```

### protein_transformer_amd/kernels.py

```python
import ctypes as C
import os

import torch

from . import _lib
from ._lib import GemmArgs, GemmHpArgs, check, lib, ptr, stream, workspace

EPI_RELU, EPI_TANH, EPI_ACCUM, EPI_GATE, EPI_SLABS = 1, 2, 4, 8, 16

GEMM_TIMING = None
GEMM_EVENT_POOL = []
GEMM_BYTES = []
GEMM_RESERVED_CUS = 0


def gemm(A, B, C_out, *, M, N, K, lda, ldb, ldc, a_kmajor=False, b_kmajor=False, bias=None, residual=None,
         ldr=0, flags=0, dropout_p=0.0, seed=0, stream_id=0, split_k=1, colsum=None, gate_scale=0.0, arith=None,
         a_scale=None, a_scale_stride=1, b_scale=None, b_scale_stride=1, gate_mask=None, ws=None):
    if ws is None:
        ws = workspace("gemm", lib().ptamd_gemm_workspace_bytes(M, N, split_k), A.device)
    args = GemmArgs(M=M, N=N, K=K, A=A.data_ptr(), lda=lda, a_kmajor=int(a_kmajor), B=B.data_ptr(), ldb=ldb,
                    b_kmajor=int(b_kmajor), C=C_out.data_ptr() if C_out is not None else ws.data_ptr(), ldc=ldc,
                    bias=bias.data_ptr() if bias is not None else None,
                    residual=residual.data_ptr() if residual is not None else None, ldr=ldr, flags=flags,
                    dropout_p=float(dropout_p), seed=int(seed) & (2 ** 64 - 1), stream_id=int(stream_id),
                    split_k=int(split_k), workspace=ws.data_ptr() if ws is not None else None,
                    workspace_bytes=ws.numel() if ws is not None else 0,
                    colsum=colsum.data_ptr() if colsum is not None else None, gate_scale=float(gate_scale),
                    arith=int(_DEFAULT_ARITH if arith is None else arith), reserved_cus=int(GEMM_RESERVED_CUS),
                    a_scale=a_scale.data_ptr() if a_scale is not None else None, a_scale_stride=int(a_scale_stride),
                    b_scale=b_scale.data_ptr() if b_scale is not None else None, b_scale_stride=int(b_scale_stride),
                    gate_mask=gate_mask.data_ptr() if gate_mask is not None else None)
    if GEMM_TIMING is None:
        check(lib().ptamd_gemm(C.byref(args), stream()), "gemm")
    else:
        e0, e1 = GEMM_EVENT_POOL.pop(), GEMM_EVENT_POOL.pop()
        e0.record()
        check(lib().ptamd_gemm(C.byref(args), stream()), "gemm")
        e1.record()
        nprod = lib().ptamd_gemm_products(C.byref(args))
        kind = "dW" if (a_kmajor and b_kmajor) else ("dX" if b_kmajor else "fwd")
        GEMM_TIMING.append((2.0 * M * N * K, e0, e1, nprod,
                            f"ptamd_gemm {kind} (staging kernel, A_KMAJOR={int(bool(a_kmajor))} B_KMAJOR={int(bool(b_kmajor))} NPROD={nprod})"))
        GEMM_BYTES.append(4 * (M * K + N * K + M * N * (1 + (residual is not None) + bool(flags & EPI_ACCUM))))
    return C_out


GEMM_F32, GEMM_BF16X3, GEMM_BF16X3_FULL, GEMM_F16X2, GEMM_AUTO = 0, 1, 2, 3, 4




def _env_arith():
    import os
    try:
        v = int(os.environ.get("PTAMD_GEMM_MODE", GEMM_AUTO))
    except ValueError:
        v = GEMM_AUTO
    return v if v in (GEMM_F32, GEMM_BF16X3, GEMM_BF16X3_FULL, GEMM_F16X2, GEMM_AUTO) else GEMM_AUTO


_DEFAULT_ARITH = _env_arith()


def set_gemm_mode(mode):
    global _DEFAULT_ARITH
    if int(mode) not in (GEMM_F32, GEMM_BF16X3, GEMM_BF16X3_FULL, GEMM_F16X2, GEMM_AUTO):
        raise ValueError(f"unknown GEMM arithmetic {mode}")
    _DEFAULT_ARITH = int(mode)


def get_gemm_mode():
    return _DEFAULT_ARITH


class HpOperand:
    __slots__ = ("planes", "scale", "rows", "K")

    def __init__(self, rows, K, device):
        self.rows, self.K = int(rows), int(K)
        self.planes = torch.empty(lib().ptamd_hp_bytes(self.rows, self.K), dtype=torch.uint8, device=device)
        self.scale = torch.empty(lib().ptamd_hp_padded_rows(self.rows), dtype=torch.float32, device=device)


def hp_split(x, transposed=False, out=None):
    assert x.dim() == 2 and x.stride(1) == 1
    rows, K = (x.shape[1], x.shape[0]) if transposed else (x.shape[0], x.shape[1])
    if out is None:
        out = HpOperand(rows, K, x.device)
    check(lib().ptamd_hp_split(ptr(x), x.stride(0), rows, K, int(transposed), ptr(out.planes), ptr(out.scale), stream()),
          "hp_split")
    return out


def gemm_hp(a, b, C_out, *, bias=None, residual=None, ldr=0, flags=0, dropout_p=0.0, seed=0, stream_id=0, split_k=1,
            gate_scale=0.0, gate_mask=None, gate_mask_out=None, kv=None, kv_col0=0, kv_heads=0):
    assert a.K == b.K
    M, N = a.rows, b.rows
    ws = workspace("gemm_hp", lib().ptamd_gemm_hp_workspace_bytes(M, N, split_k), C_out.device) if split_k > 1 else None
    args = GemmHpArgs(M=M, N=N, K=a.K, A=a.planes.data_ptr(), A_scale=a.scale.data_ptr(), B=b.planes.data_ptr(),
                      B_scale=b.scale.data_ptr(), C=C_out.data_ptr(), ldc=C_out.stride(0),
                      bias=bias.data_ptr() if bias is not None else None,
                      residual=residual.data_ptr() if residual is not None else None, ldr=ldr, flags=flags,
                      dropout_p=float(dropout_p), seed=int(seed) & (2 ** 64 - 1), stream_id=int(stream_id),
                      split_k=int(split_k), workspace=ws.data_ptr() if ws is not None else None,
                      workspace_bytes=ws.numel() if ws is not None else 0, gate_scale=float(gate_scale),
                      reserved_cus=int(GEMM_RESERVED_CUS),
                      gate_mask=gate_mask.data_ptr() if gate_mask is not None else None,
                      gate_mask_out=gate_mask_out.data_ptr() if gate_mask_out is not None else None,
                      kv_planes=kv[0].data_ptr() if kv is not None else None, kv_inv=kv[1].data_ptr() if kv is not None else None,
                      kv_col0=int(kv_col0), kv_heads=int(kv_heads))
    if GEMM_TIMING is None:
        check(lib().ptamd_gemm_hp(C.byref(args), stream()), "gemm_hp")
    else:
        e0, e1 = GEMM_EVENT_POOL.pop(), GEMM_EVENT_POOL.pop()
        e0.record()
        check(lib().ptamd_gemm_hp(C.byref(args), stream()), "gemm_hp")
        e1.record()
        GEMM_TIMING.append((2.0 * M * N * a.K, e0, e1, 3, "ptamd_gemm_hp (LDS-DMA kernel gemm_hp3_kernel, NPROD=3)"))
        GEMM_BYTES.append(4 * (M * a.K + N * a.K + M * N * (1 + (residual is not None) + bool(flags & EPI_ACCUM))))
    return C_out


DW_SLOTS = 512


def pick_split_k(M, N, K, slots=None):
    slots = DW_SLOTS if slots is None else slots
    tiles = ((M + 127) // 128) * ((N + 127) // 128)
    if tiles >= slots // 2 or K <= 512:
        return 1
    return max(1, min(K // 256, slots // tiles))


SPLIT_K_ROWS = True


def pick_split_k_rows(M, N, K, slots=256):
    tiles = ((M + 127) // 128) * ((N + 127) // 128)
    if not SPLIT_K_ROWS or tiles * 2 > slots or K < 1024:
        return 1
    return max(1, min(K // 512, slots // tiles))


def linear_fwd(x, w, b, out=None, defer_reduce=False, **epi):
    T, K = x.shape
    N = w.shape[0]
    sk = pick_split_k_rows(T, N, K)
    if defer_reduce and DEFER_REDUCE and sk > 1 and out is None and b is not None and N % 4 == 0 and N <= 512 and \
            epi.get("flags", 0) == 0 and epi.get("residual") is not None and epi.get("ldr") == N and \
            epi["residual"].is_contiguous() and int(_DEFAULT_ARITH if epi.get("arith") is None else epi["arith"]) != GEMM_F32:
        n = effective_splits(K, sk)
        if 2 <= n <= 4:
            ws = workspace("gemm_slabs", lib().ptamd_gemm_workspace_bytes(T, N, sk), x.device)
            rest = {k: v for k, v in epi.items() if k not in ("residual", "ldr", "dropout_p", "seed", "stream_id", "flags")}
            gemm(x, w, None, M=T, N=N, K=K, lda=x.stride(0), ldb=w.stride(0), ldc=N, split_k=sk, flags=EPI_SLABS, ws=ws, **rest)
            return PendingRows(Slabs(ws, n, T * N, (T, N)), b, epi["residual"], epi.get("dropout_p", 0.0), epi.get("seed", 0),
                               epi.get("stream_id", 0))
    if out is None:
        out = torch.empty(T, N, dtype=torch.float32, device=x.device)
    return gemm(x, w, out, M=T, N=N, K=K, lda=x.stride(0), ldb=w.stride(0), ldc=out.stride(0), bias=b,
                split_k=sk, **epi)


def gate_mask_buffer(M, N, device):
    return torch.empty(lib().ptamd_gate_mask_bytes(M, N) // 8, dtype=torch.int64, device=device)


class Slabs:
    __slots__ = ("buf", "n", "stride", "shape")

    def __init__(self, buf, n, stride, shape):
        self.buf, self.n, self.stride, self.shape = buf, n, stride, shape

# ... 19 lines not shown
    @property
    def shape(self):
        return self.slabs.shape

    @property
    def device(self):
        return self.residual.device


DEFER_REDUCE = os.environ.get("PTAMD_DEFER_REDUCE", "1") != "0"


def effective_splits(K, split_k):
    kblocks = -(-K // 32)
    splits = max(1, min(int(split_k), kblocks))
    per = -(-kblocks // splits) * 32
    return -(-K // per)


def linear_bwd_input(dy, w, out=None, flags=0, gate=None, gate_dropout_p=0.0, arith=None, gate_mask=None, defer_reduce=False,
                     **scales):
    T, N = dy.shape
    K = w.shape[1]
    sk = pick_split_k_rows(T, K, N)
    if defer_reduce and DEFER_REDUCE and sk > 1 and out is None and gate is None and gate_mask is None and flags == 0 and \
            K % 4 == 0 and K <= 512 and int(_DEFAULT_ARITH if arith is None else arith) != GEMM_F32:
        n = effective_splits(N, sk)
        if 2 <= n <= 4:
            ws = workspace("gemm_slabs", lib().ptamd_gemm_workspace_bytes(T, K, sk), dy.device)
            gemm(dy, w, None, M=T, N=K, K=N, lda=dy.stride(0), ldb=w.stride(0), ldc=K, b_kmajor=True, split_k=sk,
                 flags=EPI_SLABS, arith=arith, ws=ws, **scales)
            return Slabs(ws, n, T * K, (T, K))
    if out is None:
        out = torch.empty(T, K, dtype=torch.float32, device=dy.device)
    if gate_mask is not None and sk == 1 and K % 4 == 0 and out.stride(0) % 4 == 0 and out.data_ptr() % 16 == 0 and \
            int(_DEFAULT_ARITH if arith is None else arith) in (GEMM_F16X2, GEMM_AUTO) and N >= 32 and \
            dy.shape[0] * dy.stride(0) * 4 < 2 ** 32 and w.shape[0] * w.stride(0) * 4 < 2 ** 32:
        return gemm(dy, w, out, M=T, N=K, K=N, lda=dy.stride(0), ldb=w.stride(0), ldc=out.stride(0), b_kmajor=True, split_k=1,
                    flags=flags | EPI_GATE, gate_mask=gate_mask, gate_scale=1.0 / (1.0 - gate_dropout_p), arith=arith, **scales)
    if gate_mask is not None and gate is None:
        raise ValueError("linear_bwd_input: gate_mask given, but this product cannot read it (split-K, arithmetic, alignment "
                         "or operand size) and no fp32 `gate` was passed to fall back on")
    if gate is not None:
        return gemm(dy, w, out, M=T, N=K, K=N, lda=dy.stride(0), ldb=w.stride(0), ldc=out.stride(0), b_kmajor=True, split_k=sk,
                    flags=flags | EPI_GATE, residual=gate, ldr=gate.stride(0), gate_scale=1.0 / (1.0 - gate_dropout_p),
                    arith=arith, **scales)
    return gemm(dy, w, out, M=T, N=K, K=N, lda=dy.stride(0), ldb=w.stride(0), ldc=out.stride(0), b_kmajor=True, split_k=sk,
                flags=flags, arith=arith, **scales)


def linear_bwd_weight(dy, x, dw, dbias=None, arith=None, dy_scale=None, x_scale=None):
    T, N = dy.shape
    K = x.shape[1]
    if dy_scale is not None and x_scale is not None:
        return gemm(dy, x, dw, M=N, N=K, K=T, lda=dy.stride(0), ldb=x.stride(0), ldc=dw.stride(0), a_kmajor=True,
                    b_kmajor=True, flags=EPI_ACCUM, split_k=pick_split_k(N, K, T), colsum=dbias, arith=GEMM_F16X2,
                    a_scale=dy_scale, a_scale_stride=0, b_scale=x_scale, b_scale_stride=0)
    return gemm(dy, x, dw, M=N, N=K, K=T, lda=dy.stride(0), ldb=x.stride(0), ldc=dw.stride(0), a_kmajor=True,
                b_kmajor=True, flags=EPI_ACCUM, split_k=pick_split_k(N, K, T), colsum=dbias, arith=arith)


GROUP_MIN_K = int(os.environ.get("PTAMD_GROUP_MIN_K", 1024))


def pick_group_split(tiles256, T, slots=256):
    best, best_cost = 0, None
    for s in range(2, max(2, T // GROUP_MIN_K) + 1):
        rounds = -(-tiles256 * s // slots)
        cost = rounds * (-(-T // s) + 640)
        if best_cost is None or cost < best_cost:
            best, best_cost = s, cost
    return best if T >= 2048 else 0


def linear_bwd_weight_group(jobs, split_k):
    arr = (GemmArgs * len(jobs))()
    flops = 0.0
    nbytes = 0
    for j, (dy, x, dw, dbias, dy_scale, x_scale) in enumerate(jobs):
        T, N = dy.shape
        Kd = x.shape[1]
        ws = workspace(f"gemm_group{j}", lib().ptamd_gemm_workspace_bytes(N, Kd, split_k), dw.device)
        arr[j] = GemmArgs(M=N, N=Kd, K=T, A=dy.data_ptr(), lda=dy.stride(0), a_kmajor=1, B=x.data_ptr(), ldb=x.stride(0),
                          b_kmajor=1, C=dw.data_ptr(), ldc=dw.stride(0), bias=None, residual=None, ldr=0, flags=EPI_ACCUM,
                          dropout_p=0.0, seed=0, stream_id=0, split_k=int(split_k), workspace=ws.data_ptr(),
                          workspace_bytes=ws.numel(), colsum=dbias.data_ptr() if dbias is not None else None, gate_scale=0.0,
                          arith=GEMM_F16X2, reserved_cus=int(GEMM_RESERVED_CUS), a_scale=dy_scale.data_ptr(), a_scale_stride=0,
                          b_scale=x_scale.data_ptr(), b_scale_stride=0)
        flops += 2.0 * N * Kd * T
        nbytes += 4 * (N * T + Kd * T + 2 * N * Kd)
    if GEMM_TIMING is None:
        check(lib().ptamd_gemm_group(arr, len(jobs), stream()), "gemm_group")
    else:
        e0, e1 = GEMM_EVENT_POOL.pop(), GEMM_EVENT_POOL.pop()
        e0.record()
        check(lib().ptamd_gemm_group(arr, len(jobs), stream()), "gemm_group")
        e1.record()
        GEMM_TIMING.append((flops, e0, e1, 3, "ptamd_gemm_group dW (staging kernel on a group + one split-K reduce, NPROD=3)"))
        GEMM_BYTES.append(nbytes)


def colsum(x, out, accumulate=True):
    T, N = x.shape
    ws = workspace("colsum", lib().ptamd_colsum_workspace_bytes(N), x.device)
    check(lib().ptamd_colsum(ptr(x), T, N, x.stride(0), int(accumulate), ptr(out), ptr(ws), ws.numel(), stream()),
          "colsum")
    return out


def layernorm_fwd(x, gamma, beta, row_scale=None, planes=None):
    T, D = x.shape
    if isinstance(x, PendingRows):
        r = x.residual
        x.value, y = torch.empty_like(r), torch.empty_like(r)
        mean = torch.empty(T, dtype=torch.float32, device=r.device)
        rstd = torch.empty(T, dtype=torch.float32, device=r.device)
        check(lib().ptamd_layernorm_fwd_sum(ptr(x.slabs), x.slabs.n, x.slabs.stride, ptr(x.bias), ptr(r), x.dropout_p, x.seed,
                                            x.stream_id, ptr(x.value), ptr(gamma), ptr(beta), T, D, ptr(y), ptr(mean), ptr(rstd),
                                            ptr(row_scale), ptr(planes), stream()), "layernorm_fwd_sum")
        return y, mean, rstd
    y = torch.empty_like(x)
    mean = torch.empty(T, dtype=torch.float32, device=x.device)
    rstd = torch.empty(T, dtype=torch.float32, device=x.device)
    check(lib().ptamd_layernorm_fwd(ptr(x), ptr(gamma), ptr(beta), T, D, ptr(y), ptr(mean), ptr(rstd), ptr(row_scale),
                                    ptr(planes), stream()), "layernorm_fwd")
    return y, mean, rstd


def hp_view(planes, scale, rows, K):
    op = HpOperand.__new__(HpOperand)
    op.rows, op.K, op.planes = int(rows), int(K), planes
    op.scale = scale.view(torch.float32) if scale.dtype != torch.float32 else scale
    return op


def hp_split_rows(mats, outs):
    from ._lib import HpSplitJob
    for i in range(0, len(mats), 16):
        chunk = list(zip(mats[i:i + 16], outs[i:i + 16]))
        arr = (HpSplitJob * len(chunk))()
        for k, (w, o) in enumerate(chunk):
            assert w.dim() == 2 and w.stride(1) == 1 and (o.rows, o.K) == tuple(w.shape)
            assert o.scale.numel() >= lib().ptamd_hp_padded_rows(o.rows), "hp_split_rows: no room for the padding rows' scales"
            arr[k] = HpSplitJob(x=w.data_ptr(), ld=w.stride(0), rows=w.shape[0], K=w.shape[1], planes=o.planes.data_ptr(),
                                scale=o.scale.data_ptr())
        check(lib().ptamd_hp_split_rows(arr, len(chunk), stream()), "hp_split_rows")
    return outs


def hp_split_cols(mats, scales, outs):
    from ._lib import HpSplitJob
    for i in range(0, len(mats), 16):
        chunk = list(zip(mats[i:i + 16], scales[i:i + 16], outs[i:i + 16]))
        arr = (HpSplitJob * len(chunk))()
        for k, (w, sc, o) in enumerate(chunk):
            assert w.dim() == 2 and w.stride(1) == 1 and (o.rows, o.K) == (w.shape[1], w.shape[0]) and sc.numel() >= o.rows
            arr[k] = HpSplitJob(x=w.data_ptr(), ld=w.stride(0), rows=o.rows, K=o.K, planes=o.planes.data_ptr(), scale=sc.data_ptr())
        check(lib().ptamd_hp_split_cols(arr, len(chunk), stream()), "hp_split_cols")
    return outs


def _ln_workspace(D, device, pending):
    tag = "ln" if pending is None else f"ln{len(pending)}"
    return workspace(tag, lib().ptamd_layernorm_bwd_workspace_bytes(D), device)


def layernorm_bwd_flush(pending):
    from ._lib import LnReduceJob
    for i in range(0, len(pending), 16):
        chunk = pending[i:i + 16]
        arr = (LnReduceJob * len(chunk))()
        for k, (ws, D, dg, db) in enumerate(chunk):
            arr[k] = LnReduceJob(partials=ws.data_ptr(), D=D, dgamma=dg.data_ptr(), dbeta=db.data_ptr())
        check(lib().ptamd_layernorm_bwd_reduce(arr, len(chunk), stream()), "layernorm_bwd_reduce")
    del pending[:]


def layernorm_bwd_dropout(dy, x, gamma, mean, rstd, dgamma, dbeta, dres, dropout_p, seed, stream_id, row_scale=None,
                          bound_factor=None, bound_scale=None, row_scale_min=None, bound_scale_min=None, pending=None,
                          planes=None):
    T, D = x.shape
    dx = torch.empty_like(x)
    dropped = torch.empty_like(x) if dropout_p > 0 else None
    if pending is not None and len(pending) >= 16:
# ... 200 lines not shown


def onehot(seq, C):
    T = seq.numel()
    x = torch.empty(T, pad4(C), dtype=torch.float32, device=seq.device)
    check(lib().ptamd_onehot(ptr(seq), T, C, ptr(x), stream()), "onehot")
    return x


def posenc_add_fwd(x, pe, B, L, dropout_p, seed):
    y = torch.empty_like(x)
    check(lib().ptamd_posenc_add_fwd(ptr(x), ptr(pe), B, L, x.shape[1], float(dropout_p), int(seed), ptr(y), stream()),
          "posenc_add_fwd")
    return y


def posenc_add_bwd(dy, dropout_p, seed):
    dx = torch.empty_like(dy)
    check(lib().ptamd_posenc_add_bwd(ptr(dy), dy.numel(), float(dropout_p), int(seed), ptr(dx), stream()), "posenc_add_bwd")
    return dx


class WeightsPrep:

    def __init__(self, numel, segs, groups, ints, values, nstats):
        import numpy as np
        from ._lib import WprepBound, WprepPlan, WprepSeg
        dev = ints.device
        RB, PF = lib().ptamd_wprep_rows_per_block(), lib().ptamd_wprep_plain_floats_per_block()
        PANEL = 512
        segs = sorted(segs, key=lambda s: s["offset"])
        idx = lambda view, base: -1 if view is None else view.storage_offset() - base.storage_offset()
        table, blocks_a, blocks_b, plain = [], [], [], []
        ncolmax = ncolsq = 0
        pos = 0
        for s in segs:
            rows, cols, off = int(s["rows"]), int(s["cols"]), int(s["offset"])
            if cols % 4 or off % 4 or off < pos or (cols > PANEL and cols % PANEL):
                raise ValueError(f"ptamd_weights_prep: segment (offset {off}, {rows} x {cols}) is not representable")
            if off > pos:
                plain.append((pos, off - pos))
            pos = off + rows * cols
            want_cols = s.get("col_scale") is not None
            for name in ("row_planes", "col_planes"):
                if s.get(name) is not None and (rows % 32 or cols % 32):
                    raise ValueError("ptamd_weights_prep: planes need rows and cols that are multiples of 32")
            if s.get("col_planes") is not None and not want_cols:
                raise ValueError("ptamd_weights_prep: col_planes need col_scale")
            if s.get("colnorm") and (s.get("stats") is None or not want_cols):
                raise ValueError("ptamd_weights_prep: colnorm needs a statistics record and col_scale")
            stats = -1 if s.get("stats") is None else int(s["stats"])
            npanels = -(-cols // PANEL)
            wide = npanels > 1
            if wide and (s.get("row_planes") is not None or int(s.get("stats_row0", 0)) != 0):
                raise ValueError("ptamd_weights_prep: a matrix wider than 512 columns cannot have row planes or a statistics sub-range")
            colmax0 = ncolmax
            ncolmax += cols if want_cols else 0
            rowmax0 = -1
            if wide and s.get("row_scale") is not None:
                rowmax0 = ncolmax
                ncolmax += rows
            nrb = -(-rows // RB)
            for pnl in range(npanels):
                pc = min(PANEL, cols - pnl * PANEL)
                k = len(table)
                table.append(WprepSeg(
                    offset=off + pnl * PANEL, rows=rows, cols=pc, stats_row0=-1 if wide else int(s.get("stats_row0", 0)),
                    stats_index=stats, row_scale_index=-1 if wide else idx(s.get("row_scale"), ints),
                    col_scale_index=idx(s.get("col_scale"), ints) + pnl * PANEL if want_cols else -1,
                    colmax_index=colmax0 + pnl * PANEL if want_cols else 0,
                    colsq_index=ncolsq if s.get("colnorm") else -1,
                    row_planes=0 if s.get("row_planes") is None else s["row_planes"].data_ptr(), col_planes=0,
                    ld=cols, rowmax_index=rowmax0))
                blocks_a += [(k, b) for b in range(nrb)]
                if want_cols:
                    blocks_b.append((0, k, 0, 0))
                if s.get("colnorm"):
                    ncolsq += nrb * pc
            if wide and rowmax0 >= 0 or s.get("col_planes") is not None:
                k = len(table)
                table.append(WprepSeg(offset=off, rows=rows, cols=cols, stats_row0=0, stats_index=-1,
                                      row_scale_index=idx(s.get("row_scale"), ints) if wide else -1, col_scale_index=-1,
                                      colmax_index=colmax0, colsq_index=-1, row_planes=0,
                                      col_planes=0 if s.get("col_planes") is None else s["col_planes"].data_ptr(), ld=cols,
                                      rowmax_index=rowmax0))
                if rowmax0 >= 0:
                    blocks_b += [(3, k, b, 0) for b in range(-(-rows // 256))]
                if s.get("col_planes") is not None:
                    nchunks = (cols // 32) * (-(-rows // 32) * 2) * 64
                    blocks_b += [(1, k, b, 0) for b in range(-(-nchunks // 256))]
        if pos < numel:
            plain.append((pos, numel - pos))
        arr = (WprepSeg * len(table))(*table)
        n_matrix_blocks = len(blocks_a)
        for j, (first, n) in enumerate(plain):
            blocks_a += [(-(j + 1), b) for b in range(-(-n // PF))]
        by_stats = {}
        for k, t in enumerate(table):
            if t.colsq_index >= 0:
                by_stats.setdefault(int(t.stats_index), []).append(k)
        bounds, grp_rows, cn_list = [], [], []
        rec = lambda v: -1 if v is None else int(v)
        for g, jobs in enumerate(groups):
            first, cn_first = len(bounds), len(cn_list)
            for j in jobs:
                bounds.append(WprepBound(ln_gamma_stats=rec(j.get("ln_gamma")), ln_beta_stats=rec(j.get("ln_beta")), w_stats=int(j["w"]),
                                         w_stat_index=int(j["w_index"]), bias_stats=rec(j.get("bias")),
                                         sqrt_d=float(j.get("sqrt_d", 0.0)), post_scale=float(j.get("post_scale", 1.0)),
                                         out_scale=idx(j.get("out_scale"), ints), out_value=idx(j.get("out_value"), values)))
                if int(j["w_index"]) == 1 and int(j["w"]) in by_stats:
                    cn_list += [k for k in by_stats[int(j["w"])] if k not in cn_list[cn_first:]]
            grp_rows.append((first, len(bounds) - first, cn_first, len(cn_list) - cn_first))
            blocks_b.append((2, g, 0, 0))
        if not groups:
            raise ValueError("ptamd_weights_prep: at least one bounds group (it also resets the statistics)")
        up = lambda a, dt: torch.from_numpy(np.ascontiguousarray(np.asarray(a, dtype=dt))).to(dev)
        self.t_segs = torch.frombuffer(bytearray(bytes(arr)), dtype=torch.uint8).to(dev)
        self.t_blocks_a = up(blocks_a, np.int32).reshape(-1, 2)
        self.t_plain = up(plain if plain else [(0, 0)], np.int64).reshape(-1, 2)
        self.t_blocks_b = up(blocks_b, np.int32).reshape(-1, 4)
        barr = (WprepBound * max(len(bounds), 1))(*bounds)
        self.t_bounds = torch.frombuffer(bytearray(bytes(barr)), dtype=torch.uint8).to(dev)
        self.t_groups = up(grp_rows, np.int32).reshape(-1, 4)
        self.t_colnorm = up(cn_list if cn_list else [0], np.int32)
        self.colmax = torch.zeros(2, max(ncolmax, 1), dtype=torch.int32, device=dev)
        self.colsq = torch.zeros(max(ncolsq, 2), dtype=torch.float64, device=dev)
        self.stats = torch.zeros(2, nstats, 4, dtype=torch.float32, device=dev)
        self.ints, self.values = ints, values
        self.parity = 0
        self.numel = int(numel)
        self.plan = WprepPlan(segs=self.t_segs.data_ptr(), nsegs=len(table), blocks_a=self.t_blocks_a.data_ptr(),
                              nblocks_a=len(blocks_a), nblocks_a_matrices=n_matrix_blocks, plain=self.t_plain.data_ptr(),
                              nplain=len(plain), blocks_b=self.t_blocks_b.data_ptr(), nblocks_b=len(blocks_b),
                              bounds=self.t_bounds.data_ptr(), nbounds=len(bounds), groups=self.t_groups.data_ptr(),
                              ngroups=len(grp_rows), colnorm_segs=self.t_colnorm.data_ptr(), scales=ints.data_ptr(),
                              values=values.data_ptr(), colmax=self.colmax.data_ptr(), ncolmax=max(ncolmax, 1),
                              colsq=self.colsq.data_ptr(), stats=self.stats.data_ptr(), nstats=int(nstats), numel=int(numel),
                              with_planes=1)

    def _call(self, what, fn, with_planes, *args):
# ... 24 lines not shown
```

### protein_transformer_amd/models/encoder_only.py

```python
import collections
import math

import numpy as np
import torch
import torch.nn as nn

from .. import kernels as K
from ..protein.Structure import NUM_PREDICTED_ANGLES

_SITE_ATTN, _SITE_ATTN_OUT, _SITE_FFN_HID, _SITE_FFN_OUT = 0, 1, 2, 3


class _Holder(nn.Module):

    def __init__(self, **shapes):
        super().__init__()
        for name, shape in shapes.items():
            self.register_parameter(name, nn.Parameter(torch.empty(*shape)))


class _AttnHolder(nn.Module):
    def __init__(self, dm):
        super().__init__()
        for nm in ("wq", "wk", "wv", "wo"):
# ... 170 lines not shown
    def __init__(self, nlayers, nhead, dmodel, dff, max_seq_len, vocab, angle_means, use_tanh_out, dropout=0.1,
                 conv_kernel_sizes=None, conv_dim_reductions=(), use_embedding=True, conv_out_matches_dm=True):
        super().__init__()
        self.angle_means = angle_means
        self.vocab = vocab
        self.nlayers, self.nhead, self.dmodel, self.dff, self.max_seq_len = nlayers, nhead, dmodel, dff, max_seq_len
        self.use_tanh_out = use_tanh_out
        self.use_embedding = bool(use_embedding)
        self.dropout = float(dropout)
        self.attn_dropout = 0.1
        self.conv_shapes = None
        din = dmodel if self.use_embedding else len(vocab)
        self.dlayer = dmodel
        if conv_kernel_sizes is not None:
            self.conv_shapes = []
            ks, drs = list(conv_kernel_sizes), list(conv_dim_reductions)
            for i, (k, dr) in enumerate(zip(ks, drs)):
                assert k % 2 != 0, "Kernel size must be odd to maintain sequence length."
                dout = dmodel if (i == len(ks) - 1 and conv_out_matches_dm) else int(din // dr)
                self.conv_shapes.append((din, dout, k))
                din = dout
            if conv_out_matches_dm:
                self.dlayer = dmodel
            else:
                d = dmodel if self.use_embedding else len(vocab)
                for dr in drs:
                    d /= dr
                self.dlayer = int(d)
        D = self.dlayer
        assert D % nhead == 0, "The dimension of the model must be evenly divisible by the number of attn heads."
        widths = [dmodel, D, dff] + [c for _, c, _ in (self.conv_shapes or [])]
        if any(w % 4 for w in widths) or (D // nhead) not in (8, 16, 32, 64, 128):
            raise ValueError("libptamd needs channel widths that are multiples of 4 and width / n_head in {8, 16, 32, 64, 128}")
        self.encoder = _EncoderHolder(len(vocab), dmodel, D, dff, nlayers, max_seq_len, self.conv_shapes,
                                      self.use_embedding)
        self.output_projection = _Holder(weight=(NUM_PREDICTED_ANGLES * 2, D), bias=(NUM_PREDICTED_ANGLES * 2,))
        self._flat = None
        self._flat_grad = None
        self._layout = self._make_layout()
        self.dropout_seed = 0x5DEECE66D
        self._step_counter = 0
        self.grad_hook = None
        self.attn_row_scales = True
        self.attn_mode = None
        self.gemm_mode = None
        self.hp_forward = True
        self.hp_qkv = True
        self.keep_attn_bits = True
        self.ffn_gate_mask = True
        self.hp_dx = True
        self.side_stream_dw = True
        self.top_layer_scales = True
        self.dw_group = "auto"
        self.kv_planes = True
        self.weights_prep = True
        self.auto_guard = AutoGuard(nlayers)
        self._init_parameters()

    def _make_layout(self):
        order = ["encoder.input_embedding.emb.weight"] if self.use_embedding else []
        for j in range(len(self.conv_shapes or [])):
            order += [f"encoder.conv_layers.{j}.weight", f"encoder.conv_layers.{j}.bias"]
        for i in range(self.nlayers):
            b = f"encoder.enc_layers.{i}."
            order += [b + f"self_attn.{n}.weight" for n in ("wq", "wk", "wv")]
            order += [b + f"self_attn.{n}.bias" for n in ("wq", "wk", "wv")]
            order += [b + "self_attn.wo.weight", b + "self_attn.wo.bias",
                      b + "pwff.layer1.weight", b + "pwff.layer1.bias", b + "pwff.layer2.weight", b + "pwff.layer2.bias",
                      b + "sublayer_connections.0.norm.weight", b + "sublayer_connections.0.norm.bias",
                      b + "sublayer_connections.1.norm.weight", b + "sublayer_connections.1.norm.bias"]
        order += ["output_projection.weight", "output_projection.bias"]
        params = dict(self.named_parameters())
        assert set(order) == set(params)
        layout, off = {}, 0
        for name in order:
            shape = tuple(params[name].shape)
            layout[name] = (off, shape)
            off += (int(np.prod(shape)) + 3) // 4 * 4
        self._flat_numel = off
        return layout

    def _init_parameters(self):
        for name, p in self.named_parameters():
            if p.dim() > 1:
                nn.init.xavier_uniform_(p)
            elif "norm.weight" in name:
                nn.init.ones_(p)
            elif "norm.bias" in name:
                nn.init.zeros_(p)
            elif "conv_layers" in name:
                ci, _, k = self.conv_shapes[int(name.split(".")[2])]
                nn.init.uniform_(p, -1 / math.sqrt(ci * k), 1 / math.sqrt(ci * k))
            else:
                fan_in = self.dff if "layer2" in name else self.dlayer
                nn.init.uniform_(p, -1 / math.sqrt(fan_in), 1 / math.sqrt(fan_in))
        am = np.asarray(self.angle_means, dtype=np.float64)
        if self.use_tanh_out:
            am = np.arctanh(am)
        with torch.no_grad():
            self.output_projection.bias.copy_(torch.tensor(am, dtype=torch.float32))
            self.output_projection.weight.zero_()

    def _ensure_flat(self):
        fast = self.__dict__.get("_flat_fast")
        if fast is not None:
            flat, first, last, off_last, gfirst = fast
# ... 138 lines not shown
            W = lambda name: self._slice(flat, name)
            for i in range(self.nlayers):
                b = f"encoder.enc_layers.{i}."
                wqkv, bqkv = self._qkv(flat, i)
                L = dict(rs_qkv=take(3 * D), cs_qkv=take(D), rs_o=take(D), cs_o=take(D), rs_1p=take(Fp), cs_1=take(D),
                         rs_2=take(D), cs_2=take(F), att_scale=take(4), f1_scale=take(4), h1_scale=take(4), h2_scale=take(4),
                         dqkv_scale=take(4), dz1_factor=factor[i, 2:3], dz1_factor_rec=factor[i])
                L["rs_1"] = L["rs_1p"][:F]
                L.update(dy2_min=minbuf[i, 0:4], dz1_min=minbuf[i, 4:8], dyo_min=minbuf[i, 8:12], dqkv_min=minbuf[i, 12:16])
                st = stats[i]
                wjobs += [dict(w=wqkv, row_scale=L["rs_qkv"], col_scale=L["cs_qkv"]),
                          dict(w=wqkv[2 * D:], stats=st[0]),
                          dict(w=W(b + "self_attn.wo.weight"), row_scale=L["rs_o"], col_scale=L["cs_o"]),
                          dict(w=W(b + "pwff.layer1.weight"), row_scale=L["rs_1"], col_scale=L["cs_1"], stats=st[1]),
                          dict(w=W(b + "pwff.layer2.weight"), row_scale=L["rs_2"], col_scale=L["cs_2"], stats=st[2]),
                          dict(w=W(b + "sublayer_connections.0.norm.weight"), stats=st[3]),
                          dict(w=W(b + "sublayer_connections.0.norm.bias"), stats=st[4]),
                          dict(w=W(b + "sublayer_connections.1.norm.weight"), stats=st[5]),
                          dict(w=W(b + "sublayer_connections.1.norm.bias"), stats=st[6]),
                          dict(w=bqkv[2 * D:], stats=st[7]),
                          dict(w=W(b + "pwff.layer1.bias"), stats=st[8])]
                sq = math.sqrt(D)
                bjobs += [dict(ln_gamma=st[3], ln_beta=st[4], w=st[0], w_index=0, bias=st[7], sqrt_d=sq,
                               post_scale=1.0 / (1.0 - pa), out_scale=L["att_scale"]),
                          dict(ln_gamma=st[5], ln_beta=st[6], w=st[1], w_index=0, bias=st[8], sqrt_d=sq,
                               post_scale=1.0 / (1.0 - p), out_scale=L["f1_scale"]),
                          dict(w=st[2], w_index=1, post_scale=1.0 / (1.0 - p), out_value=L["dz1_factor"]),
                          dict(ln_gamma=st[3], ln_beta=st[4], w=ones, w_index=0, sqrt_d=sq, out_scale=L["h1_scale"]),
                          dict(ln_gamma=st[5], ln_beta=st[6], w=ones, w_index=0, sqrt_d=sq, out_scale=L["h2_scale"])]
                layers.append(L)
            assert o == n_i
            dq_stats = torch.zeros(self.nlayers, 4, dtype=torch.float32, device=dev)
            gstats = torch.zeros(self.nlayers, len(AutoGuard.SITES), 4, dtype=torch.float32, device=dev)
            for i, L in enumerate(layers):
                L["dqkv_stats"] = dq_stats[i]
                L["minbuf"] = minbuf
                L["guard_stats"], L["ints"] = gstats, ints
                L["top_stats"] = top_stats
            cache = caches[key] = dict(layers=layers, wjobs=wjobs, bjobs=bjobs,
                                       keep=(ints, stats, factor, ones, dq_stats, minbuf, gstats, top_stats))
            cache["hp_mats"], cache["hp_outs"] = [], []
            cache["hpT_mats"], cache["hpT_scales"], cache["hpT_outs"] = [], [], []
            if D % 32 == 0 and D <= 2048:
                for i, L in enumerate(layers):
                    w1 = W(f"encoder.enc_layers.{i}.pwff.layer1.weight")
                    L["hp_1"] = K.hp_view(torch.empty(K.lib().ptamd_hp_bytes(F, D), dtype=torch.uint8, device=dev), L["rs_1p"], F, D)
                    L["hp_qkv"] = K.hp_view(torch.empty(K.lib().ptamd_hp_bytes(3 * D, D), dtype=torch.uint8, device=dev),
                                            L["rs_qkv"], 3 * D, D)
                    cache["hp_mats"] += [w1, self._qkv(flat, i)[0]]
                    cache["hp_outs"] += [L["hp_1"], L["hp_qkv"]]
                    w2 = W(f"encoder.enc_layers.{i}.pwff.layer2.weight")
                    planes2 = torch.empty(K.lib().ptamd_hp_bytes(F, D), dtype=torch.uint8, device=dev)
                    L["hp_2t"] = K.hp_view(planes2, L["cs_2"], F, D)
                    cache["hpT_mats"] += [w2]
                    cache["hpT_scales"] += [L["cs_2"]]
                    cache["hpT_outs"] += [L["hp_2t"]]
            panels_ok = all(c <= 512 or c % 512 == 0 for c in (D, F))
            cache["prep"] = self._build_prep(cache, p, pa) if (F <= 2048 and D % 4 == 0 and F % 4 == 0 and panels_ok) else None
        need_planes = bool(cache["hp_mats"]) and bool(hp)
        if self.weights_prep and cache.get("prep") is not None:
            stamp = self._weights_stamp()
            fresh = cache.get("fresh")
            if fresh is None or fresh[0] != stamp or (need_planes and not fresh[1]):
                cache["prep"].prepare(self._flat, with_planes=need_planes)
                cache["fresh"] = (stamp, need_planes)
                self.__dict__["_prep_launches"] = self.__dict__.get("_prep_launches", 0) + 1
            if self.training and backward:
                self.__dict__["_train_cache"] = (cache, need_planes)
            return cache["layers"]
        K.weight_scales(cache["wjobs"])
        K.bound_scales(cache["bjobs"])
        if cache["hp_mats"] and hp:
            if self.hp_qkv:
                K.hp_split_rows(cache["hp_mats"], cache["hp_outs"])
            else:
                K.hp_split_rows(cache["hp_mats"][0::2], cache["hp_outs"][0::2])
            if self.hp_dx and F % 32 == 0 and backward:
                K.hp_split_cols(cache["hpT_mats"], cache["hpT_scales"], cache["hpT_outs"])
        return cache["layers"]

    def _build_prep(self, cache, p, pa):
        D, F = self.dlayer, self.dff
        layers = cache["layers"]
        ints, factor = cache["keep"][0], cache["keep"][2]
        off = lambda name: self._layout[name][0]
        planes_ok = bool(cache["hp_mats"])
        segs, groups = [], []
        for i, L in enumerate(layers):
            b = f"encoder.enc_layers.{i}."
            r = lambda k, i=i: 9 * i + k
            segs += [
                dict(offset=off(b + "self_attn.wq.weight"), rows=3 * D, cols=D, row_scale=L["rs_qkv"], col_scale=L["cs_qkv"],
                     stats=r(0), stats_row0=2 * D, row_planes=L["hp_qkv"].planes if planes_ok else None),
                dict(offset=off(b + "self_attn.wq.bias") + 2 * D, rows=1, cols=D, stats=r(7)),
                dict(offset=off(b + "self_attn.wo.weight"), rows=D, cols=D, row_scale=L["rs_o"], col_scale=L["cs_o"]),
                dict(offset=off(b + "pwff.layer1.weight"), rows=F, cols=D, row_scale=L["rs_1"], col_scale=L["cs_1"], stats=r(1),
                     row_planes=L["hp_1"].planes if planes_ok else None),
                dict(offset=off(b + "pwff.layer1.bias"), rows=1, cols=F, stats=r(8)),
                dict(offset=off(b + "pwff.layer2.weight"), rows=D, cols=F, row_scale=L["rs_2"], col_scale=L["cs_2"], stats=r(2),
                     colnorm=True, col_planes=L["hp_2t"].planes if (planes_ok and F % 32 == 0) else None),
                dict(offset=off(b + "sublayer_connections.0.norm.weight"), rows=1, cols=D, stats=r(3)),
                dict(offset=off(b + "sublayer_connections.0.norm.bias"), rows=1, cols=D, stats=r(4)),
                dict(offset=off(b + "sublayer_connections.1.norm.weight"), rows=1, cols=D, stats=r(5)),
                dict(offset=off(b + "sublayer_connections.1.norm.bias"), rows=1, cols=D, stats=r(6))]
            sq = math.sqrt(D)
            groups.append([
                dict(ln_gamma=r(3), ln_beta=r(4), w=r(0), w_index=0, bias=r(7), sqrt_d=sq, post_scale=1.0 / (1.0 - pa),
                     out_scale=L["att_scale"]),
                dict(ln_gamma=r(5), ln_beta=r(6), w=r(1), w_index=0, bias=r(8), sqrt_d=sq, post_scale=1.0 / (1.0 - p),
                     out_scale=L["f1_scale"]),
                dict(w=r(2), w_index=1, post_scale=1.0 / (1.0 - p), out_value=L["dz1_factor"]),
                dict(ln_gamma=r(3), ln_beta=r(4), w=-1, w_index=0, sqrt_d=sq, out_scale=L["h1_scale"]),
                dict(ln_gamma=r(5), ln_beta=r(6), w=-1, w_index=0, sqrt_d=sq, out_scale=L["h2_scale"])])
        return K.WeightsPrep(self._flat_numel, segs, groups, ints, factor.view(-1), 9 * self.nlayers)

    def _slice(self, buf, name):
        cache = self.__dict__.setdefault("_view_cache", {})
        ptr = buf.data_ptr()
        key = (ptr, name)
        v = cache.get(key)
        if v is None:
            off, shape = self._layout[name]
            v = buf[off:off + int(np.prod(shape))].view(shape)
            if (self._flat is not None and ptr == self._flat.data_ptr()) or \
                    (self._flat_grad is not None and ptr == self._flat_grad.data_ptr()):
                cache[key] = v.detach()
                v = cache[key]
        return v

    def _qkv(self, buf, i):
        cache = self.__dict__.setdefault("_view_cache", {})
        key = (buf.data_ptr(), "qkv", i)
        v = cache.get(key)
        if v is None:
            b = f"encoder.enc_layers.{i}.self_attn."
            off_w, _ = self._layout[b + "wq.weight"]
            off_b, _ = self._layout[b + "wq.bias"]
            D = self.dlayer
            v = (buf[off_w:off_w + 3 * D * D].view(3 * D, D).detach(), buf[off_b:off_b + 3 * D].detach())
            if (self._flat is not None and key[0] == self._flat.data_ptr()) or \
                    (self._flat_grad is not None and key[0] == self._flat_grad.data_ptr()):
                cache[key] = v
        return v

    def forward(self, enc_input, dec_input=None):
        flat, _ = self._ensure_flat()
        if enc_input.shape[1] > self.max_seq_len:
            raise RuntimeError(f"sequence length {enc_input.shape[1]} exceeds max_seq_len={self.max_seq_len} "
                               "(the reference's positional table has the same limit, Sublayers.py:48,60)")
        seq = enc_input.to(flat.device, torch.int64).contiguous()
        if self.training:
            self._step_counter += 1
        seed = (self.dropout_seed + 0x9E3779B97F4A7C15 * self._step_counter) & (2 ** 63 - 1)
# ... 2 lines not shown
        return out.view(seq.shape[0], seq.shape[1], NUM_PREDICTED_ANGLES * 2)

    def predict(self, enc_input):
        return self.forward(enc_input)

    def set_dropout(self, p, attn_p=None):
        self.dropout = float(p)
        self.attn_dropout = float(p if attn_p is None else attn_p)


class _PassPlan:
    def __init__(self, m, seq, seed, backward):
        (B, L), D = seq.shape, m.dlayer
        self.B, self.L, self.D, self.H, self.backward, self.seed = B, L, D, m.nhead, backward, seed
        self.p, self.pa = (m.dropout, m.attn_dropout) if m.training else (0.0, 0.0)
        self.arith = ar = K.get_gemm_mode() if m.gemm_mode is None else int(m.gemm_mode)
        self.attn_arith = ar if m.attn_mode is None else int(m.attn_mode)
        if ar == K.GEMM_AUTO and B * L * D < AUTO_F16X2_MIN_WORK:
            self.arith = K.GEMM_BF16X3
        self.fuse = D <= 1024
        self.side = None
        if backward and m.side_stream_dw and D >= 512 and B * L >= SIDE_STREAM_MIN_TOKENS and B * L * D <= SIDE_STREAM_MAX_WORK:
            if m.__dict__.get("_side_stream") is None or m._side_stream.device != seq.device:
                m.__dict__["_side_stream"] = torch.cuda.Stream(device=seq.device)
            self.side = m._side_stream
        self.dw_group = m.dw_group
        if self.dw_group == "auto":
            ffn_tiles = -(-D // 256) * -(-m.dff // 128) + -(-m.dff // 256) * -(-D // 128)
            self.dw_group = "pairs" if ffn_tiles * B * L >= 256 * 2048 else "layer"

    def take_scales(self, m, flat):
        B, L, D, H, attn = self.B, self.L, self.D, self.H, self.attn_arith
        want_hp = B * L >= HP_MIN_TOKENS and bool(m.hp_forward)
        scales = self.scales = m._step_scales(flat, self.arith, self.p, self.pa, hp=want_hp, backward=self.backward)
        self.use_hp = want_hp and scales is not None and "hp_1" in scales[0]
        self.hp_qkv = self.use_hp and m.hp_qkv
        self.kv_planes = self.hp_qkv and m.kv_planes and K.attention_reads_kv_planes(B, L, H, D // H, attn)
        self.keep_bits = self.pa > 0.0 and m.keep_attn_bits and self.backward and K.attention_bwd_reads_keep_bits(B, L, H, D // H, attn)
        self.gate_mask = m.ffn_gate_mask and self.backward
        self.hp_dx = self.use_hp and m.hp_dx and self.fuse and "hp_2t" in scales[0] and m.dff % 32 == 0
        self.attn_row_scales = scales is not None and m.attn_row_scales and K.attention_row_scales_available(D // H, attn)
        self.top_scales = scales is not None and self.fuse and m.top_layer_scales
        guard = self.guard = m.auto_guard if (scales is not None and m.auto_guard.enabled) else None
        self.measure, self.measure_fwd, self.off, self.wide = False, False, None, None
        if guard is not None:
            guard.poll()
            if m.training and self.backward:
                self.measure = guard.want_measure()
                guard.count_step()
            else:
                self.measure_fwd = guard.want_measure_forward()
                guard.eval_passes += 1
            self.off, self.wide = guard.off.copy(), guard.wide.copy()

    def prod(self, i, k, **scale_kw):
        if self.wide is not None and self.wide[i, k]:
            return dict(arith=K.GEMM_BF16X3)
        return dict(arith=self.arith, **scale_kw)


_Acts = collections.namedtuple("_Acts", "x mean1 rstd1 h1 qkv att lse x2 mean2 rstd2 h2 f1 kbits fmask kv")


def _layer_fwd(plan, m, flat, seq, i, x, hplanes):
    Tn, D, H, p, seed, dev = plan.B * plan.L, plan.D, plan.H, plan.p, plan.seed, x.device
    W = lambda name: m._slice(flat, name)
    b = f"encoder.enc_layers.{i}."
    sid = i * 8
    sc = plan.scales[i] if plan.scales is not None else None
    wqkv, bqkv = m._qkv(flat, i)
    s_h1 = torch.empty(Tn, dtype=torch.int32, device=dev) if sc else None
    hp_q = plan.hp_qkv and not (plan.wide is not None and plan.wide[i, 0])
    h1, mean1, rstd1 = K.layernorm_fwd(x, W(b + "sublayer_connections.0.norm.weight"),
                                       W(b + "sublayer_connections.0.norm.bias"), row_scale=s_h1,
                                       planes=hplanes if hp_q else None)
    if isinstance(x, K.PendingRows):
        x = x.value
    kv = None
    if hp_q and plan.kv_planes:
        kv = K.attention_kv_buffers(Tn, H, dev)
        m.__dict__["_kv_plane_passes"] = m.__dict__.get("_kv_plane_passes", 0) + 1
    if hp_q:
        qkv = K.gemm_hp(K.hp_view(hplanes, s_h1, Tn, D), sc["hp_qkv"],
                        torch.empty(Tn, 3 * D, dtype=torch.float32, device=dev), bias=bqkv, kv=kv, kv_col0=D, kv_heads=H)
    else:
        qkv = K.linear_fwd(h1, wqkv, bqkv, **plan.prod(i, 0, a_scale=s_h1, b_scale=sc and sc["rs_qkv"]))
    kbits = None
    if plan.keep_bits:
        kbits = K.attention_keep_bits(plan.B, plan.L, H, dev)
        m.__dict__["_attn_bits_passes"] = m.__dict__.get("_attn_bits_passes", 0) + 1
    att, lse = K.attention_fwd(qkv, seq, H, plan.pa, seed, sid + _SITE_ATTN, arith=plan.attn_arith, keep_bits=kbits, kv=kv)
    use_b = sc is not None and not (plan.off is not None and plan.off[i, 0])
    x2 = K.linear_fwd(att, W(b + "self_attn.wo.weight"), W(b + "self_attn.wo.bias"), residual=x, ldr=D,
                      dropout_p=p, seed=seed, stream_id=sid + _SITE_ATTN_OUT,
                      **plan.prod(i, 1, a_scale=sc["att_scale"] if use_b else None, a_scale_stride=0 if use_b else 1,
                                  b_scale=sc and sc["rs_o"]))
    s_h2 = torch.empty(Tn, dtype=torch.int32, device=dev) if sc else None
    h2, mean2, rstd2 = K.layernorm_fwd(x2, W(b + "sublayer_connections.1.norm.weight"),
                                       W(b + "sublayer_connections.1.norm.bias"), row_scale=s_h2, planes=hplanes)
    fmask = None
    if plan.use_hp and not (plan.wide is not None and plan.wide[i, 2]):
        if plan.gate_mask:
            fmask = K.gate_mask_buffer(Tn, m.dff, dev)
            m.__dict__["_gate_mask_passes"] = m.__dict__.get("_gate_mask_passes", 0) + 1
        f1 = K.gemm_hp(K.hp_view(hplanes, s_h2, Tn, D), sc["hp_1"],
                       torch.empty(Tn, m.dff, dtype=torch.float32, device=dev), bias=W(b + "pwff.layer1.bias"),
                       flags=K.EPI_RELU, dropout_p=p, seed=seed, stream_id=sid + _SITE_FFN_HID, gate_mask_out=fmask)
    else:
        f1 = K.linear_fwd(h2, W(b + "pwff.layer1.weight"), W(b + "pwff.layer1.bias"), flags=K.EPI_RELU,
                          dropout_p=p, seed=seed, stream_id=sid + _SITE_FFN_HID,
                          **plan.prod(i, 2, a_scale=s_h2, b_scale=sc and sc["rs_1"]))
    use_b = sc is not None and not (plan.off is not None and plan.off[i, 1])
    x3 = K.linear_fwd(f1, W(b + "pwff.layer2.weight"), W(b + "pwff.layer2.bias"), residual=x2, ldr=D,
                      dropout_p=p, seed=seed, stream_id=sid + _SITE_FFN_OUT, defer_reduce=i + 1 < m.nlayers,
                      **plan.prod(i, 3, a_scale=sc["f1_scale"] if use_b else None, a_scale_stride=0 if use_b else 1,
                                  b_scale=sc and sc["rs_2"]))
    if plan.measure_fwd:
        gs = sc["guard_stats"][i]
        K.weight_scales([dict(w=t, stats=gs[j], rows_only=True) for j, t in ((0, att), (1, f1), (3, h1), (4, h2))])
    return x3, _Acts(x, mean1, rstd1, h1, qkv, att, lse, x2, mean2, rstd2, h2, f1, kbits, fmask, kv)


class _GradSchedule:
    def __init__(self, model, plan, main):
        self.model, self.side, self.group, self.main = model, plan.side, plan.dw_group, main
        self.queue = []
        self.ln_pending = []
        self.keep = []

    def run(self, fn, *args, keep=(), **kw):
        if self.side is None:
            return fn(*args, **kw)
        self.side.wait_stream(self.main)
        self.keep.extend(keep)
        with torch.cuda.stream(self.side):
            return fn(*args, **kw)

    def later(self, dy, x, gw, gb, arith=None, dy_scale=None, x_scale=None):
        if self.group == "off":
            return self.run(K.linear_bwd_weight, dy, x, gw, gb, keep=(dy, x), arith=arith, dy_scale=dy_scale, x_scale=x_scale)
        self.queue.append((dy, x, gw, gb, arith, dy_scale, x_scale))

    def flush(self):
        jobs, self.queue = self.queue, []
        ok = [j for j in jobs if j[5] is not None and j[6] is not None and j[1].shape[1] % 4 == 0]
        tiles = sum(-(-j[0].shape[1] // 256) * -(-j[1].shape[1] // 128) for j in ok)
        sk = K.pick_group_split(tiles, ok[0][0].shape[0]) if 2 <= len(ok) <= 4 else 0
        if sk < 2:
            ok = []
        for dy, x, gw, gb, a, sy, sx in jobs:
            if not any(dy is o[0] and x is o[1] for o in ok):
                self.run(K.linear_bwd_weight, dy, x, gw, gb, keep=(dy, x), arith=a, dy_scale=sy, x_scale=sx)
        if ok:
            group = [(dy, x, gw, gb, sy, sx) for dy, x, gw, gb, a, sy, sx in ok]
            self.run(K.linear_bwd_weight_group, group, sk, keep=(t for j in ok for t in j[:2]))

    def join(self):
        if self.side is not None:
            self.main.wait_stream(self.side)
            self.keep.clear()

    def done(self, first, last):
        hook = self.model.grad_hook
        if hook is not None:
            K.layernorm_bwd_flush(self.ln_pending)
            self.run(hook, *self.model._span(first, last))


def _layer_bwd(plan, m, flat, gflat, seq, i, a, carry, dws, s_dqkv_all, dy2_planes):
    dx, dy2, s_dy2, bs_dz1, have_min, have_planes = carry
    D, H, p, pa, seed, ar, fuse, dev = plan.D, plan.H, plan.p, plan.pa, plan.seed, plan.arith, plan.fuse, dx.device
    W = lambda name: m._slice(flat, name)
    G = lambda name: m._slice(gflat, name)
    i32 = lambda: torch.empty(plan.B * plan.L, dtype=torch.int32, device=dev)
    scales, wide = plan.scales, plan.wide
    b = f"encoder.enc_layers.{i}."
    sid = i * 8
    sc = scales[i] if scales is not None else None
    if dy2 is None:
        dy2 = K.dropout_bwd(dx, p, seed, sid + _SITE_FFN_OUT) if p > 0 else dx
        if plan.top_scales:
            ts = sc["top_stats"]
            K.weight_scales([dict(w=dy2, stats=ts, rows_only=True)])
            K.bound_scales([dict(w=ts, w_index=2, out_scale=sc["dy2_min"]),
                            dict(ln_gamma=sc["dz1_factor_rec"], sqrt_d=1.0, w=ts, w_index=0, out_scale=sc["dz1_min"])])
            have_min = True
    uni = sc is not None and have_min
    o_att, o_f1, o_dz1, o_h1, o_h2 = (bool(v) for v in plan.off[i]) if plan.off is not None else (False,) * 5
    dws.later(dy2, a.f1, G(b + "pwff.layer2.weight"), G(b + "pwff.layer2.bias"), arith=ar,
              dy_scale=sc["dy2_min"] if uni and not o_f1 else None, x_scale=sc["f1_scale"] if uni and not o_f1 else None)
    if dy2_planes is not None and have_planes and not (wide is not None and wide[i, 7]):
        dz1 = K.gemm_hp(K.hp_view(dy2_planes, s_dy2, plan.B * plan.L, D), sc["hp_2t"],
                        torch.empty(plan.B * plan.L, m.dff, dtype=torch.float32, device=dev),
                        residual=a.f1 if a.fmask is None else None, ldr=a.f1.stride(0) if a.fmask is None else 0,
                        gate_mask=a.fmask, flags=K.EPI_GATE, gate_scale=1.0 / (1.0 - p))
    else:
        dz1 = K.linear_bwd_input(dy2, W(b + "pwff.layer2.weight"), gate=a.f1, gate_dropout_p=p, gate_mask=a.fmask,
                                 **plan.prod(i, 7, a_scale=s_dy2 if sc else None, b_scale=sc and sc["cs_2"]))
    if plan.measure:
        gs = sc["guard_stats"][i]
        K.weight_scales([dict(w=t, stats=gs[j], rows_only=True) for j, t in enumerate((a.att, a.f1, dz1, a.h1, a.h2))])
    uni1 = uni and not (o_dz1 or o_h2)
    dws.later(dz1, a.h2, G(b + "pwff.layer1.weight"), G(b + "pwff.layer1.bias"), arith=ar,
              dy_scale=sc["dz1_min"] if uni1 else None, x_scale=sc["h2_scale"] if uni1 else None)
    if dws.group != "layer":
        dws.flush()
    dh2 = K.linear_bwd_input(dz1, W(b + "pwff.layer1.weight"), defer_reduce=fuse,
                             **plan.prod(i, 6, a_scale=bs_dz1 if sc and not o_dz1 else None, b_scale=sc and sc["cs_1"]))
    g2w, g2b = G(b + "sublayer_connections.1.norm.weight"), G(b + "sublayer_connections.1.norm.bias")
    if fuse:
        s_dyo = i32() if sc else None
        dx2, dyo = K.layernorm_bwd_dropout(dh2, a.x2, W(b + "sublayer_connections.1.norm.weight"), a.mean2, a.rstd2, g2w, g2b,
                                           dx, p, seed, sid + _SITE_ATTN_OUT, row_scale=s_dyo,
                                           row_scale_min=sc["dyo_min"] if sc else None, pending=dws.ln_pending)
    else:
        s_dyo = None
        dx2 = K.layernorm_bwd(dh2, a.x2, W(b + "sublayer_connections.1.norm.weight"), a.mean2, a.rstd2, g2w, g2b, dres=dx,
                              pending=dws.ln_pending)
        dyo = K.dropout_bwd(dx2, p, seed, sid + _SITE_ATTN_OUT) if p > 0 else dx2
    uni_o = sc is not None and fuse and not o_att
    dws.later(dyo, a.att, G(b + "self_attn.wo.weight"), G(b + "self_attn.wo.bias"), arith=ar,
              dy_scale=sc["dyo_min"] if uni_o else None, x_scale=sc["att_scale"] if uni_o else None)
    datt = K.linear_bwd_input(dyo, W(b + "self_attn.wo.weight"), **plan.prod(i, 5, a_scale=s_dyo, b_scale=sc and sc["cs_o"]))
    s_dqkv = s_dqkv_all[i] if plan.attn_row_scales else None
    dqkv = K.attention_bwd(a.qkv, seq, a.att, datt, a.lse, H, pa, seed, sid + _SITE_ATTN, arith=plan.attn_arith,
                           row_scale=s_dqkv, row_scale_min=sc["dqkv_min"] if plan.attn_row_scales else None, keep_bits=a.kbits,
                           kv=a.kv)
    gw, gb = m._qkv(gflat, i)
    dq_uni = sc["dqkv_min"] if sc is not None else None
    if sc is not None and not plan.attn_row_scales:
        s_dqkv, dq_uni = i32(), sc["dqkv_scale"]
        K.weight_scales([dict(w=dqkv, row_scale=s_dqkv, stats=sc["dqkv_stats"], rows_only=True)])
        K.bound_scales([dict(w=sc["dqkv_stats"], w_index=2, out_scale=sc["dqkv_scale"])])
    uni_h1 = sc is not None and not o_h1
    dws.later(dqkv, a.h1, gw, gb, arith=ar, dy_scale=dq_uni if uni_h1 else None, x_scale=sc["h1_scale"] if uni_h1 else None)
    dh1 = K.linear_bwd_input(dqkv, m._qkv(flat, i)[0], defer_reduce=fuse and i > 0,
                             **plan.prod(i, 4, a_scale=s_dqkv, b_scale=sc and sc["cs_qkv"]))
    g1w, g1b = G(b + "sublayer_connections.0.norm.weight"), G(b + "sublayer_connections.0.norm.bias")
    if fuse and i > 0:
        s_dy2, bs_dz1 = (i32(), i32()) if scales is not None else (None, None)
        below = scales[i - 1] if scales is not None else None
        dx, dy2 = K.layernorm_bwd_dropout(dh1, a.x, W(b + "sublayer_connections.0.norm.weight"), a.mean1, a.rstd1, g1w, g1b,
                                          dx2, p, seed, (i - 1) * 8 + _SITE_FFN_OUT, row_scale=s_dy2,
                                          bound_factor=below["dz1_factor"] if below else None, bound_scale=bs_dz1,
                                          row_scale_min=below["dy2_min"] if below else None,
                                          bound_scale_min=below["dz1_min"] if below else None, pending=dws.ln_pending,
                                          planes=dy2_planes if below else None)
        have_min = below is not None
        have_planes = below is not None and dy2_planes is not None
    else:
# ... 107 lines not shown
```

Baseline: 1.580 million residues/s.

## Write FFN hidden activations directly as f16 hi/lo planes and consume them in FFN2

The FFN first GEMM epilogue can now emit the ReLU/dropout hidden activation straight into pre-split f16 hi/lo plane blocks with a uniform scale, instead of a full f32 tensor. The second FFN GEMM reads those planes plus a new pre-split row-plane copy of the layer2 weight that weight prep builds, and the weight-gradient GEMM can take B operands already in plane form. The aim is to remove the f32 write/read of the large Tn x dff hidden tensor and the per-tile splitting work in FFN2 and its dW. The cost is extra weight-prep work and plane buffers, plus an added constraint that the forward gate mask must be available in backward.

```diff
diff --git a/include/ptamd.h b/include/ptamd.h
--- a/include/ptamd.h
+++ b/include/ptamd.h
@@ -80,6 +80,7 @@
   const uint32_t *a_scale; int a_scale_stride;
   const uint32_t *b_scale; int b_scale_stride;
   const uint64_t *gate_mask;
+  int b_hp_planes;
 } ptamd_gemm_args;
 size_t ptamd_gate_mask_bytes(int M, int N);
 size_t ptamd_gemm_workspace_bytes(int M, int N, int split_k);
@@ -118,6 +119,8 @@
   const uint64_t *gate_mask;
   uint64_t *gate_mask_out;
   void *kv_planes; float *kv_inv; int kv_col0, kv_heads;
+  int a_scale_uniform;
+  void *c_planes; const float *c_scale;
 } ptamd_gemm_hp_args;
 size_t ptamd_gemm_hp_workspace_bytes(int M, int N, int split_k);
 int ptamd_gemm_hp(const ptamd_gemm_hp_args *args, void *stream);
diff --git a/protein_transformer_amd/_lib.py b/protein_transformer_amd/_lib.py
--- a/protein_transformer_amd/_lib.py
+++ b/protein_transformer_amd/_lib.py
@@ -32,7 +32,8 @@
                 ("reserved_cus", _i),
                 ("a_scale", _p), ("a_scale_stride", _i),
                 ("b_scale", _p), ("b_scale_stride", _i),
-                ("gate_mask", _p)]
+                ("gate_mask", _p),
+                ("b_hp_planes", _i)]
 
 
 class WScaleJob(C.Structure):
@@ -71,7 +72,8 @@
                 ("gate_scale", _f),
                 ("reserved_cus", _i),
                 ("gate_mask", _p), ("gate_mask_out", _p),
-                ("kv_planes", _p), ("kv_inv", _p), ("kv_col0", _i), ("kv_heads", _i)]
+                ("kv_planes", _p), ("kv_inv", _p), ("kv_col0", _i), ("kv_heads", _i),
+                ("a_scale_uniform", _i), ("c_planes", _p), ("c_scale", _p)]
 
 
 class WprepSeg(C.Structure):
diff --git a/protein_transformer_amd/csrc/gemm.hip b/protein_transformer_amd/csrc/gemm.hip
--- a/protein_transformer_amd/csrc/gemm.hip
+++ b/protein_transformer_amd/csrc/gemm.hip
@@ -405,6 +405,10 @@
   if (a->gate_mask && !(a->flags & PTAMD_EPI_GATE)) return PTAMD_ERR_BAD_SHAPE;
   p.gate_mask = a->gate_mask; p.gate_mask_out = nullptr;
   p.mask_rb = (a->M + 31) / 32; p.mask_cb = (a->N + 31) / 32;
+  p.b_planes = a->b_hp_planes != 0;
+  if (p.b_planes && (!a->a_kmajor || !a->b_kmajor || (a->K & 31) || (a->N & 127) || a->ldb != a->N || !a->b_scale ||
+                     a->b_scale_stride != 0 || a->arith != PTAMD_GEMM_F16X2))
+    return PTAMD_ERR_BAD_SHAPE;
   user_c = a->C;
   if (splits > 1) {
     if (!a->workspace || a->workspace_bytes < slab_bytes(a->M, a->N, splits)) return PTAMD_ERR_WORKSPACE;
@@ -413,6 +417,7 @@
     if (a->colsum) p.colsum = p.C + (size_t)splits * p.slab;
   }
   mode = resolve_mode(a);
+  if (p.b_planes && mode != PTAMD_GEMM_F16X2) return PTAMD_ERR_BAD_SHAPE;
   if (a->gate_mask && (mode != PTAMD_GEMM_F16X2 || !p.vec_epilogue || splits > 1 || a->dropout_p != 0.f)) return PTAMD_ERR_BAD_SHAPE;
   p.scale_a = p.scale_b = nullptr;
   p.scale_a_stride = p.scale_b_stride = 1;
diff --git a/protein_transformer_amd/csrc/gemm_common.h b/protein_transformer_amd/csrc/gemm_common.h
--- a/protein_transformer_amd/csrc/gemm_common.h
+++ b/protein_transformer_amd/csrc/gemm_common.h
@@ -37,6 +37,7 @@
   const uint64_t *gate_mask;
   uint64_t *gate_mask_out;
   int mask_rb, mask_cb;
+  int b_planes;
 };
 __device__ __forceinline__ uint32_t load_gate_masks(const GemmParams &p, int rb, int cb, int lane) {
   const int rbu = __builtin_amdgcn_readfirstlane(rb), cbu = __builtin_amdgcn_readfirstlane(cb);
diff --git a/protein_transformer_amd/csrc/gemm_hp.hip b/protein_transformer_amd/csrc/gemm_hp.hip
--- a/protein_transformer_amd/csrc/gemm_hp.hip
+++ b/protein_transformer_amd/csrc/gemm_hp.hip
@@ -25,6 +25,10 @@
   char *kv_planes;
   float *kv_inv;
   int kv_col0, kv_heads, kv_nt;
+  int a_stride;
+  char *c_planes;
+  const float *c_scale;
+  int c_kb16, c_rows_p;
 };
 
 typedef __attribute__((address_space(1))) const void *gptr_t;
@@ -184,7 +188,7 @@
           for (int g = 0; g < 4; ++g)
 #pragma unroll
             for (int e = 0; e < 4; ++e) {
-              const float ia = inverse_of_scale(p.a_scale[min(row0 + i * 32 + 8 * g + 4 * lh + e, p.g.M - 1)]);
+              const float ia = inverse_of_scale(p.a_scale[min(row0 + i * 32 + 8 * g + 4 * lh + e, p.g.M - 1) * p.a_stride]);
 #pragma unroll
               for (int j = 0; j < 2; ++j) acc[i][j][g * 4 + e] = acc[i][j][g * 4 + e] * ia * ib[j];
             }
@@ -212,7 +216,7 @@
 
 typedef HpGeom<4, 2, 2, true> Geom;
 
-template <int EPI, bool KVP = false>
+template <int EPI, bool KVP = false, bool CPL = false>
 int launch_hp3(const HpParams &p, int splits, hipStream_t st);
 template <int EPI>
 int launch_hp(const HpParams &p, int splits, hipStream_t st) {
@@ -246,7 +250,7 @@
   return v;
 }
 
-template <int EPI, bool KVP = false>
+template <int EPI, bool KVP = false, bool CPL = false>
 __device__ __forceinline__ void hp3_epilogue(const GemmParams &p, const f32x16 (&acc)[2][2], float *C, int ldc, bool partial,
                                              int row0, int col0, int lane, uint32_t thr, float keep_scale, float *scratch,
                                              const HpParams *hp = nullptr) {
@@ -341,6 +345,21 @@
         }
         continue;
       }
+      if (CPL) {
+        const int kbl = lane >> 4, q = lane & 15, rr = q >> 1, h = (q & 1) ^ (g & 1);
+        const int row = row0 + i * 32 + 8 * g + rr;
+        float4 a = *reinterpret_cast<const float4 *>(scratch + rr * 64 + kbl * 16 + h * 8);
+        float4 b = *reinterpret_cast<const float4 *>(scratch + rr * 64 + kbl * 16 + h * 8 + 4);
+        if (row >= p.M) a = b = make_float4(0.f, 0.f, 0.f, 0.f);
+        uint4 hi, lo;
+        kv_split8(a, b, hp->c_scale[0], hi, lo);
+        if (row < hp->c_rows_p && col0 < p.N) {
+          char *dst = hp->c_planes + block_offset((row0 >> 5) + i, (col0 >> 4) + kbl, 0, hp->c_kb16) + (16 * g + q) * 16;
+          *reinterpret_cast<uint4 *>(dst) = hi;
+          *reinterpret_cast<uint4 *>(dst + BLK_BYTES) = lo;
+        }
+        continue;
+      }
 #pragma unroll
       for (int u = 0; u < 2; ++u) {
         const int f = lane + 64 * u, rr = f >> 4, c4 = (f & 15) * 4;
@@ -385,7 +404,7 @@
 
 #define PT_DS_READ_B128(dst, addr, off) asm volatile("ds_read_b128 %0, %1 offset:%2" : "=v"(dst) : "v"(addr), "n"(off))
 
-template <int EPI, bool KVP = false>
+template <int EPI, bool KVP = false, bool CPL = false>
 __global__ __launch_bounds__(Hp3::THREADS, 2) void gemm_hp3_kernel(const HpParams p) {
   using G = Hp3;
   extern __shared__ __attribute__((aligned(16))) char smem[];
@@ -525,12 +544,12 @@
           for (int g = 0; g < 4; ++g)
 #pragma unroll
             for (int e = 0; e < 4; ++e) {
-              const float ia = inverse_of_scale(p.a_scale[min(row0 + i * 32 + 8 * g + 4 * lh + e, p.g.M - 1)]);
+              const float ia = inverse_of_scale(p.a_scale[min(row0 + i * 32 + 8 * g + 4 * lh + e, p.g.M - 1) * p.a_stride]);
 #pragma unroll
               for (int j = 0; j < 2; ++j) acc[i][j][g * 4 + e] = acc[i][j][g * 4 + e] * ia * ib[j];
             }
       }
-      hp3_epilogue<EPI, KVP>(p.g, acc, C, ldc, partial, row0, col0, lane, thr, keep_scale, scratch + wave * 512, &p);
+      hp3_epilogue<EPI, KVP, CPL>(p.g, acc, C, ldc, partial, row0, col0, lane, thr, keep_scale, scratch + wave * 512, &p);
       zero_acc();
     }
     if (!advance(cc)) break;
@@ -538,10 +557,10 @@
   }
 }
 
-template <int EPI, bool KVP>
+template <int EPI, bool KVP, bool CPL>
 int launch_hp3(const HpParams &p, int splits, hipStream_t st) {
   const int work = ((p.g.M + Hp3::TILE_M - 1) / Hp3::TILE_M) * ((p.g.N + HBN - 1) / HBN) * splits;
-  auto kern = gemm_hp3_kernel<EPI, KVP>;
+  auto kern = gemm_hp3_kernel<EPI, KVP, CPL>;
   PT_HIP_TRY(hipFuncSetAttribute(reinterpret_cast<const void *>(kern), hipFuncAttributeMaxDynamicSharedMemorySize, (int)Hp3::LDS));
   const int slots = ptgemm::persistent_grid(p.g.reserved_cus);
   hipLaunchKernelGGL(kern, dim3(work < slots ? work : slots), dim3(Hp3::THREADS), Hp3::LDS, st, p);
@@ -789,7 +808,7 @@
 
 int ptamd_gemm_hp(const ptamd_gemm_hp_args *a, void *stream) {
   if (!a || a->M <= 0 || a->N <= 0 || a->K <= 0) return PTAMD_ERR_BAD_SHAPE;
-  if (!a->A || !a->B || !a->A_scale || !a->B_scale || !a->C) return PTAMD_ERR_BAD_SHAPE;
+  if (!a->A || !a->B || !a->A_scale || !a->B_scale || (!a->C && !a->c_planes)) return PTAMD_ERR_BAD_SHAPE;
   if (!pt_aligned16(a->A) || !pt_aligned16(a->B)) return PTAMD_ERR_ALIGN;
   if (a->dropout_p < 0.f || a->dropout_p >= 1.f) return PTAMD_ERR_BAD_SHAPE;
   if ((a->flags & PTAMD_EPI_GATE) && (a->residual == nullptr) == (a->gate_mask == nullptr)) return PTAMD_ERR_BAD_SHAPE;
@@ -804,6 +823,11 @@
   g.colsum = nullptr; g.colsum_share = 1; g.scale_a = g.scale_b = nullptr; g.scale_a_stride = g.scale_b_stride = 1;
   g.gate_mask = a->gate_mask; g.gate_mask_out = a->gate_mask_out;
   g.mask_rb = (a->M + 31) / 32; g.mask_cb = (a->N + 31) / 32;
+  g.b_planes = 0;
+  if ((a->flags & PTAMD_EPI_SLABS) && (a->bias || a->residual || a->gate_mask || a->gate_mask_out || a->kv_planes || a->c_planes ||
+                                      a->dropout_p != 0.f || (a->flags & ~PTAMD_EPI_SLABS)))
+    return PTAMD_ERR_BAD_SHAPE;
+  g.flags = a->flags & ~PTAMD_EPI_SLABS;
   constexpr int HBK = 32;
   const int Kp = round_up(a->K, 32), stages = Kp / HBK;
   int splits = a->split_k > 1 ? a->split_k : 1;
@@ -832,7 +856,19 @@
   p.kv_col0 = a->kv_col0;
   p.kv_heads = a->kv_heads;
   p.kv_nt = a->M / 32;
+  p.a_stride = a->a_scale_uniform ? 0 : 1;
+  p.c_planes = static_cast<char *>(a->c_planes);
+  p.c_scale = a->c_scale;
+  p.c_kb16 = round_up(a->N, 32) / 16;
+  p.c_rows_p = round_up(a->M, 32);
   hipStream_t st = (hipStream_t)stream;
+  if (a->c_planes) {
+    if (!a->c_scale || (a->N & 63) || !g.vec_epilogue || splits > 1 || a->residual || a->gate_mask || a->kv_planes ||
+        (a->flags & ~PTAMD_EPI_RELU))
+      return PTAMD_ERR_BAD_SHAPE;
+    if (!pt_aligned16(a->c_planes)) return PTAMD_ERR_ALIGN;
+    return launch_hp3<ptgemm::EPI_FULL, false, true>(p, 1, st);
+  }
   if (a->kv_planes) {
     if (!a->kv_inv || a->kv_heads <= 0 || (a->M & 31) || (a->kv_col0 & 63) || a->kv_col0 < 0 ||
         a->N != a->kv_col0 + 2 * a->kv_heads * 64 || !g.vec_epilogue || splits > 1 || a->residual || a->gate_mask ||
@@ -848,7 +884,7 @@
   if (plain || splits > 1) rc = launch_hp<ptgemm::EPI_PLAIN>(p, splits, st);
   else if (a->dropout_p == 0.f) rc = launch_hp<ptgemm::EPI_NODROP>(p, splits, st);
   else rc = launch_hp<ptgemm::EPI_FULL>(p, splits, st);
-  if (rc || splits == 1) return rc;
+  if (rc || splits == 1 || (a->flags & PTAMD_EPI_SLABS)) return rc;
   const float *slabs = g.C;
   g.C = user_c;
   return ptgemm::launch_splitk_reduce(g, slabs, splits, nullptr, nullptr, st);
diff --git a/protein_transformer_amd/csrc/gemm_split_kernel.h b/protein_transformer_amd/csrc/gemm_split_kernel.h
--- a/protein_transformer_amd/csrc/gemm_split_kernel.h
+++ b/protein_transformer_amd/csrc/gemm_split_kernel.h
@@ -133,6 +133,18 @@
 #pragma unroll
   for (int i = 0; i < NV; ++i) store_split_f16_one<G, KMAJOR, ROWS>(s, pt, v[i], sc, i);
 }
+template <int NV>
+__device__ __forceinline__ void plane_item_offsets(int r0, int pt, uint32_t (&voff)[NV]) {
+#pragma unroll
+  for (int i = 0; i < NV; ++i) voff[i] = (uint32_t)(r0 >> 4) * 2048u + (uint32_t)(pt + NPRODUCER * i) * 16u;
+}
+template <typename G, int ROWS>
+__device__ __forceinline__ void store_planes_one(unsigned short *__restrict__ s, int pt, const float4 &v, int i) {
+  constexpr int PLANE = G::template plane<ROWS>(), LD_KR = ROWS + KR_PAD;
+  const int q = pt + NPRODUCER * i, blk = q >> 6, c = q & 63;
+  const int kl = c >> 1, h = (c & 1) ^ ((kl >> 3) & 1);
+  *reinterpret_cast<float4 *>(s + (blk & 1) * PLANE + kl * LD_KR + (blk >> 1) * 16 + h * 8) = v;
+}
 __device__ __forceinline__ uint32_t row_scale_bits(uint32_t amax) { return min(268u - (amax >> 23), 254u) << 23; }
 __device__ __forceinline__ float inverse_scale(uint32_t scale_bits) { return __uint_as_float((254u << 23) - scale_bits); }
 
@@ -181,6 +193,7 @@
   float *const cs_area = scratch + SCRATCH_FLOATS;
 
   constexpr bool F16 = NPROD == 3;
+  constexpr bool BPL = F16 && A_KMAJOR && B_KMAJOR && TI == 4;
   const int tid = threadIdx.x, lane = tid & 63, wave = tid >> 6;
   auto P = [&](int j) __attribute__((always_inline)) -> const GemmParams & {
     if constexpr (GROUPED) return arg.p[j];
@@ -244,8 +257,12 @@
     uint32_t voa[NVA], vob[NVB];
     const float *opA = P(ld.it.pj).A, *opB = P(ld.it.pj).B;
     int op_lda = P(ld.it.pj).lda, op_ldb = P(ld.it.pj).ldb;
+    auto offsets_b = [&]() __attribute__((always_inline)) {
+      if (BPL && P(ld.it.pj).b_planes) plane_item_offsets<NVB>(ld.it.bn0, pt, vob);
+      else item_offsets<G, B_KMAJOR, TBN>(op_ldb, P(ld.it.pj).N, ld.it.bn0, pt, vob);
+    };
     item_offsets<G, A_KMAJOR, TBM>(op_lda, P(ld.it.pj).M, ld.it.bm0, pt, voa);
-    item_offsets<G, B_KMAJOR, TBN>(op_ldb, P(ld.it.pj).N, ld.it.bn0, pt, vob);
+    offsets_b();
     float4 ra[NSETS][NVA], rb[NSETS][NVB];
     float rsa[NSETS][MAX_NV], rsb[NSETS][MAX_NV];
     uint32_t soa[MAX_NV], sob[MAX_NV];
@@ -267,7 +284,7 @@
           op_lda = P(ld.it.pj).lda; op_ldb = P(ld.it.pj).ldb;
         }
         item_offsets<G, A_KMAJOR, TBM>(op_lda, P(ld.it.pj).M, ld.it.bm0, pt, voa);
-        item_offsets<G, B_KMAJOR, TBN>(op_ldb, P(ld.it.pj).N, ld.it.bn0, pt, vob);
+        offsets_b();
         if (F16) {
           scale_offsets<G, A_KMAJOR, TBM>(P(ld.it.pj).M, ld.it.bm0, pt, soa, P(ld.it.pj).scale_a_stride);
           scale_offsets<G, B_KMAJOR, TBN>(P(ld.it.pj).N, ld.it.bn0, pt, sob, P(ld.it.pj).scale_b_stride);
@@ -301,6 +318,7 @@
         const float *na = opA + (A_KMAJOR ? (size_t)ks_next * op_lda : (size_t)ks_next);
         const float *nb = opB + (B_KMAJOR ? (size_t)ks_next * op_ldb : (size_t)ks_next);
         constexpr int GRP = 2;
+        const bool b_pre = BPL && P(st.it.pj).b_planes;
 #pragma unroll
         for (int i0 = 0; i0 < NVA; i0 += GRP) {
 #pragma unroll
@@ -314,7 +332,10 @@
 #pragma unroll
         for (int i0 = 0; i0 < NVB; i0 += GRP) {
 #pragma unroll
-          for (int i = i0; i < i0 + GRP && i < NVB; ++i) store_split_f16_one<G, B_KMAJOR, TBN>(sb, pt, b[i], sb_, i);
+          for (int i = i0; i < i0 + GRP && i < NVB; ++i) {
+            if (BPL && b_pre) store_planes_one<G, TBN>(sb, pt, b[i], i);
+            else store_split_f16_one<G, B_KMAJOR, TBN>(sb, pt, b[i], sb_, i);
+          }
           __builtin_amdgcn_sched_barrier(0);
 #pragma unroll
           for (int i = i0; i < i0 + GRP && i < NVB; ++i)
diff --git a/protein_transformer_amd/csrc/wprep.hip b/protein_transformer_amd/csrc/wprep.hip
--- a/protein_transformer_amd/csrc/wprep.hip
+++ b/protein_transformer_amd/csrc/wprep.hip
@@ -257,6 +257,32 @@
       pl.scales[sg.row_scale_index + r] = pt_row_scale_bits(pl.colmax[sg.rowmax_index + r]);
       pl.colmax_next[sg.rowmax_index + r] = 0u;
     }
+    return;
+  }
+  if (blk.x == 4) {
+    if (!pl.with_planes) return;
+    const ptamd_wprep_seg sg = pl.segs[blk.y];
+    const int kbv = sg.cols >> 4;
+    const int64_t nchunks = (int64_t)(sg.rows / 32) * kbv * 64;
+    const int64_t id = (int64_t)blk.z * 256 + tid;
+    if (id >= nchunks) return;
+    const int c = (int)(id & 63);
+    const int64_t b = id >> 6;
+    const int kb = (int)(b % kbv), rb = (int)(b / kbv);
+    int r, h;
+    pthp::chunk_coords(c, r, h);
+    const int row = rb * 32 + r;
+    const float sc = __uint_as_float(pt_row_scale_bits(pl.colmax[sg.rowmax_index + row]));
+    const float *x = w + sg.offset + (int64_t)row * sg.ld + kb * 16 + h * 8;
+    const float4 a = *reinterpret_cast<const float4 *>(x), q = *reinterpret_cast<const float4 *>(x + 4);
+    uint4 hi, lo;
+    ptsplit::split_pair_f16(a.x, a.y, sc, sc, hi.x, lo.x);
+    ptsplit::split_pair_f16(a.z, a.w, sc, sc, hi.y, lo.y);
+    ptsplit::split_pair_f16(q.x, q.y, sc, sc, hi.z, lo.z);
+    ptsplit::split_pair_f16(q.z, q.w, sc, sc, hi.w, lo.w);
+    char *dst = reinterpret_cast<char *>(sg.row_planes) + pthp::block_offset(rb, kb, 0, kbv) + c * 16;
+    *reinterpret_cast<uint4 *>(dst) = hi;
+    *reinterpret_cast<uint4 *>(dst + pthp::BLK_BYTES) = lo;
     return;
   }
   if (blk.x == 1) {
diff --git a/protein_transformer_amd/kernels.py b/protein_transformer_amd/kernels.py
--- a/protein_transformer_amd/kernels.py
+++ b/protein_transformer_amd/kernels.py
@@ -16,7 +16,7 @@
 
 def gemm(A, B, C_out, *, M, N, K, lda, ldb, ldc, a_kmajor=False, b_kmajor=False, bias=None, residual=None,
          ldr=0, flags=0, dropout_p=0.0, seed=0, stream_id=0, split_k=1, colsum=None, gate_scale=0.0, arith=None,
-         a_scale=None, a_scale_stride=1, b_scale=None, b_scale_stride=1, gate_mask=None, ws=None):
+         a_scale=None, a_scale_stride=1, b_scale=None, b_scale_stride=1, gate_mask=None, ws=None, b_hp_planes=0):
     if ws is None:
         ws = workspace("gemm", lib().ptamd_gemm_workspace_bytes(M, N, split_k), A.device)
     args = GemmArgs(M=M, N=N, K=K, A=A.data_ptr(), lda=lda, a_kmajor=int(a_kmajor), B=B.data_ptr(), ldb=ldb,
@@ -30,7 +30,7 @@
                     arith=int(_DEFAULT_ARITH if arith is None else arith), reserved_cus=int(GEMM_RESERVED_CUS),
                     a_scale=a_scale.data_ptr() if a_scale is not None else None, a_scale_stride=int(a_scale_stride),
                     b_scale=b_scale.data_ptr() if b_scale is not None else None, b_scale_stride=int(b_scale_stride),
-                    gate_mask=gate_mask.data_ptr() if gate_mask is not None else None)
+                    gate_mask=gate_mask.data_ptr() if gate_mask is not None else None, b_hp_planes=int(b_hp_planes))
     if GEMM_TIMING is None:
         check(lib().ptamd_gemm(C.byref(args), stream()), "gemm")
     else:
@@ -75,12 +75,30 @@
 
 
 class HpOperand:
-    __slots__ = ("planes", "scale", "rows", "K")
+    __slots__ = ("planes", "scale", "rows", "K", "uniform")
 
     def __init__(self, rows, K, device):
         self.rows, self.K = int(rows), int(K)
+        self.uniform = False
         self.planes = torch.empty(lib().ptamd_hp_bytes(self.rows, self.K), dtype=torch.uint8, device=device)
         self.scale = torch.empty(lib().ptamd_hp_padded_rows(self.rows), dtype=torch.float32, device=device)
+
+    @property
+    def shape(self):
+        return (self.rows, self.K)
+
+    def dense(self):
+        rb, kb = -(-self.rows // 32), -(-self.K // 32) * 2
+        t = self.planes[:rb * kb * 2048].view(torch.float16).view(rb, kb, 2, 32, 2, 8).float()
+        t = t[:, :, 0] + t[:, :, 1]
+        swap = ((torch.arange(32, device=t.device) >> 3) & 1).bool()
+        t = torch.where(swap.view(1, 1, 32, 1, 1), t.flip(3), t)
+        x = t.permute(0, 2, 1, 3, 4).reshape(rb * 32, kb * 16)[:self.rows, :self.K]
+        s = self.scale.view(torch.float32)
+        return x / (s[0] if self.uniform else s[:self.rows].unsqueeze(1))
+
+    def view(self, *shape):
+        return self.dense().view(*shape)
 
 
 def hp_split(x, transposed=False, out=None):
@@ -94,12 +112,20 @@
 
 
 def gemm_hp(a, b, C_out, *, bias=None, residual=None, ldr=0, flags=0, dropout_p=0.0, seed=0, stream_id=0, split_k=1,
-            gate_scale=0.0, gate_mask=None, gate_mask_out=None, kv=None, kv_col0=0, kv_heads=0):
-    assert a.K == b.K
+            gate_scale=0.0, gate_mask=None, gate_mask_out=None, kv=None, kv_col0=0, kv_heads=0, out_planes=None, ws=None):
+    assert a.K == b.K and not b.uniform
     M, N = a.rows, b.rows
-    ws = workspace("gemm_hp", lib().ptamd_gemm_hp_workspace_bytes(M, N, split_k), C_out.device) if split_k > 1 else None
+    dev = a.planes.device
+    if ws is None and split_k > 1:
+        ws = workspace("gemm_hp", lib().ptamd_gemm_hp_workspace_bytes(M, N, split_k), dev)
+    if out_planes is not None:
+        assert C_out is None and out_planes.uniform and (out_planes.rows, out_planes.K) == (M, N)
+    c_ptr = C_out.data_ptr() if C_out is not None else (ws.data_ptr() if ws is not None and out_planes is None else None)
     args = GemmHpArgs(M=M, N=N, K=a.K, A=a.planes.data_ptr(), A_scale=a.scale.data_ptr(), B=b.planes.data_ptr(),
-                      B_scale=b.scale.data_ptr(), C=C_out.data_ptr(), ldc=C_out.stride(0),
+                      B_scale=b.scale.data_ptr(), C=c_ptr, ldc=C_out.stride(0) if C_out is not None else N,
+                      a_scale_uniform=int(a.uniform),
+                      c_planes=out_planes.planes.data_ptr() if out_planes is not None else None,
+                      c_scale=out_planes.scale.data_ptr() if out_planes is not None else None,
                       bias=bias.data_ptr() if bias is not None else None,
                       residual=residual.data_ptr() if residual is not None else None, ldr=ldr, flags=flags,
                       dropout_p=float(dropout_p), seed=int(seed) & (2 ** 64 - 1), stream_id=int(stream_id),
@@ -119,7 +145,23 @@
         e1.record()
         GEMM_TIMING.append((2.0 * M * N * a.K, e0, e1, 3, "ptamd_gemm_hp (LDS-DMA kernel gemm_hp3_kernel, NPROD=3)"))
         GEMM_BYTES.append(4 * (M * a.K + N * a.K + M * N * (1 + (residual is not None) + bool(flags & EPI_ACCUM))))
-    return C_out
+    return out_planes if out_planes is not None else C_out
+
+
+def linear_fwd_hp(a, b, bias, defer_reduce=False, **epi):
+    T, K, N = a.rows, a.K, b.rows
+    dev = a.planes.device
+    sk = pick_split_k_rows(T, N, K)
+    if defer_reduce and DEFER_REDUCE and sk > 1 and bias is not None and N % 4 == 0 and N <= 512 and \
+            epi.get("flags", 0) == 0 and epi.get("residual") is not None and epi.get("ldr") == N and epi["residual"].is_contiguous():
+        n = effective_splits(K, sk)
+        if 2 <= n <= 4:
+            ws = workspace("gemm_slabs", lib().ptamd_gemm_hp_workspace_bytes(T, N, sk), dev)
+            gemm_hp(a, b, None, split_k=sk, flags=EPI_SLABS, ws=ws)
+            return PendingRows(Slabs(ws, n, T * N, (T, N)), bias, epi["residual"], epi.get("dropout_p", 0.0), epi.get("seed", 0),
+                               epi.get("stream_id", 0))
+    out = torch.empty(T, N, dtype=torch.float32, device=dev)
+    return gemm_hp(a, b, out, bias=bias, split_k=sk, **epi)
 
 
 DW_SLOTS = 512
@@ -245,6 +287,12 @@
 def linear_bwd_weight(dy, x, dw, dbias=None, arith=None, dy_scale=None, x_scale=None):
     T, N = dy.shape
     K = x.shape[1]
+    if isinstance(x, HpOperand):
+        if dy_scale is None or not x.uniform:
+            raise ValueError("linear_bwd_weight: a pre-split x needs uniform scales on both operands (there is no fp32 x to fall back on)")
+        return gemm(dy, x.planes, dw, M=N, N=K, K=T, lda=dy.stride(0), ldb=K, ldc=dw.stride(0), a_kmajor=True,
+                    b_kmajor=True, flags=EPI_ACCUM, split_k=pick_split_k(N, K, T), colsum=dbias, arith=GEMM_F16X2,
+                    a_scale=dy_scale, a_scale_stride=0, b_scale=x.scale, b_scale_stride=0, b_hp_planes=1)
     if dy_scale is not None and x_scale is not None:
         return gemm(dy, x, dw, M=N, N=K, K=T, lda=dy.stride(0), ldb=x.stride(0), ldc=dw.stride(0), a_kmajor=True,
                     b_kmajor=True, flags=EPI_ACCUM, split_k=pick_split_k(N, K, T), colsum=dbias, arith=GEMM_F16X2,
@@ -274,12 +322,16 @@
         T, N = dy.shape
         Kd = x.shape[1]
         ws = workspace(f"gemm_group{j}", lib().ptamd_gemm_workspace_bytes(N, Kd, split_k), dw.device)
-        arr[j] = GemmArgs(M=N, N=Kd, K=T, A=dy.data_ptr(), lda=dy.stride(0), a_kmajor=1, B=x.data_ptr(), ldb=x.stride(0),
+        pre = isinstance(x, HpOperand)
+        if pre:
+            assert x.uniform
+            x, x_scale = x.planes, x.scale
+        arr[j] = GemmArgs(M=N, N=Kd, K=T, A=dy.data_ptr(), lda=dy.stride(0), a_kmajor=1, B=x.data_ptr(), ldb=Kd if pre else x.stride(0),
                           b_kmajor=1, C=dw.data_ptr(), ldc=dw.stride(0), bias=None, residual=None, ldr=0, flags=EPI_ACCUM,
                           dropout_p=0.0, seed=0, stream_id=0, split_k=int(split_k), workspace=ws.data_ptr(),
                           workspace_bytes=ws.numel(), colsum=dbias.data_ptr() if dbias is not None else None, gate_scale=0.0,
                           arith=GEMM_F16X2, reserved_cus=int(GEMM_RESERVED_CUS), a_scale=dy_scale.data_ptr(), a_scale_stride=0,
-                          b_scale=x_scale.data_ptr(), b_scale_stride=0)
+                          b_scale=x_scale.data_ptr(), b_scale_stride=0, b_hp_planes=int(pre))
         flops += 2.0 * N * Kd * T
         nbytes += 4 * (N * T + Kd * T + 2 * N * Kd)
     if GEMM_TIMING is None:
@@ -320,9 +372,9 @@
     return y, mean, rstd
 
 
-def hp_view(planes, scale, rows, K):
+def hp_view(planes, scale, rows, K, uniform=False):
     op = HpOperand.__new__(HpOperand)
-    op.rows, op.K, op.planes = int(rows), int(K), planes
+    op.rows, op.K, op.planes, op.uniform = int(rows), int(K), planes, bool(uniform)
     op.scale = scale.view(torch.float32) if scale.dtype != torch.float32 else scale
     return op
 
@@ -629,8 +681,11 @@
             stats = -1 if s.get("stats") is None else int(s["stats"])
             npanels = -(-cols // PANEL)
             wide = npanels > 1
-            if wide and (s.get("row_planes") is not None or int(s.get("stats_row0", 0)) != 0):
-                raise ValueError("ptamd_weights_prep: a matrix wider than 512 columns cannot have row planes or a statistics sub-range")
+            if wide and int(s.get("stats_row0", 0)) != 0:
+                raise ValueError("ptamd_weights_prep: a matrix wider than 512 columns cannot have a statistics sub-range")
+            if wide and s.get("row_planes") is not None and s.get("row_scale") is None:
+                raise ValueError("ptamd_weights_prep: row_planes of a matrix wider than 512 columns need row_scale")
+            wide_planes = s["row_planes"] if wide and s.get("row_planes") is not None else None
             colmax0 = ncolmax
             ncolmax += cols if want_cols else 0
             rowmax0 = -1
@@ -647,7 +702,7 @@
                     col_scale_index=idx(s.get("col_scale"), ints) + pnl * PANEL if want_cols else -1,
                     colmax_index=colmax0 + pnl * PANEL if want_cols else 0,
                     colsq_index=ncolsq if s.get("colnorm") else -1,
-                    row_planes=0 if s.get("row_planes") is None else s["row_planes"].data_ptr(), col_planes=0,
+                    row_planes=0 if (wide or s.get("row_planes") is None) else s["row_planes"].data_ptr(), col_planes=0,
                     ld=cols, rowmax_index=rowmax0))
                 blocks_a += [(k, b) for b in range(nrb)]
                 if want_cols:
@@ -658,11 +713,14 @@
                 k = len(table)
                 table.append(WprepSeg(offset=off, rows=rows, cols=cols, stats_row0=0, stats_index=-1,
                                       row_scale_index=idx(s.get("row_scale"), ints) if wide else -1, col_scale_index=-1,
-                                      colmax_index=colmax0, colsq_index=-1, row_planes=0,
+                                      colmax_index=colmax0, colsq_index=-1,
+                                      row_planes=0 if wide_planes is None else wide_planes.data_ptr(),
                                       col_planes=0 if s.get("col_planes") is None else s["col_planes"].data_ptr(), ld=cols,
                                       rowmax_index=rowmax0))
                 if rowmax0 >= 0:
                     blocks_b += [(3, k, b, 0) for b in range(-(-rows // 256))]
+                if wide_planes is not None:
+                    blocks_b += [(4, k, b, 0) for b in range(-(-((rows // 32) * (cols // 16) * 64) // 256))]
                 if s.get("col_planes") is not None:
                     nchunks = (cols // 32) * (-(-rows // 32) * 2) * 64
                     blocks_b += [(1, k, b, 0) for b in range(-(-nchunks // 256))]
diff --git a/protein_transformer_amd/models/encoder_only.py b/protein_transformer_amd/models/encoder_only.py
--- a/protein_transformer_amd/models/encoder_only.py
+++ b/protein_transformer_amd/models/encoder_only.py
@@ -246,6 +246,7 @@
         self.side_stream_dw = True
         self.top_layer_scales = True
         self.dw_group = "auto"
+        self.ffn_hidden_planes = True
         self.kv_planes = True
         self.weights_prep = True
         self.auto_guard = AutoGuard(nlayers)
@@ -490,6 +491,8 @@
                     w2 = W(f"encoder.enc_layers.{i}.pwff.layer2.weight")
                     planes2 = torch.empty(K.lib().ptamd_hp_bytes(F, D), dtype=torch.uint8, device=dev)
                     L["hp_2t"] = K.hp_view(planes2, L["cs_2"], F, D)
+                    if F % 32 == 0:
+                        L["hp_2"] = K.hp_view(torch.empty(K.lib().ptamd_hp_bytes(D, F), dtype=torch.uint8, device=dev), L["rs_2"], D, F)
                     cache["hpT_mats"] += [w2]
                     cache["hpT_scales"] += [L["cs_2"]]
                     cache["hpT_outs"] += [L["hp_2t"]]
@@ -505,7 +508,9 @@
                 self.__dict__["_prep_launches"] = self.__dict__.get("_prep_launches", 0) + 1
             if self.training and backward:
                 self.__dict__["_train_cache"] = (cache, need_planes)
+            cache["layers"][0]["hp_2_valid"] = need_planes and "hp_2" in cache["layers"][0]
             return cache["layers"]
+        cache["layers"][0]["hp_2_valid"] = False
         K.weight_scales(cache["wjobs"])
         K.bound_scales(cache["bjobs"])
         if cache["hp_mats"] and hp:
@@ -536,7 +541,8 @@
                      row_planes=L["hp_1"].planes if planes_ok else None),
                 dict(offset=off(b + "pwff.layer1.bias"), rows=1, cols=F, stats=r(8)),
                 dict(offset=off(b + "pwff.layer2.weight"), rows=D, cols=F, row_scale=L["rs_2"], col_scale=L["cs_2"], stats=r(2),
-                     colnorm=True, col_planes=L["hp_2t"].planes if (planes_ok and F % 32 == 0) else None),
+                     colnorm=True, col_planes=L["hp_2t"].planes if (planes_ok and F % 32 == 0) else None,
+                     row_planes=L["hp_2"].planes if (planes_ok and "hp_2" in L) else None),
                 dict(offset=off(b + "sublayer_connections.0.norm.weight"), rows=1, cols=D, stats=r(3)),
                 dict(offset=off(b + "sublayer_connections.0.norm.bias"), rows=1, cols=D, stats=r(4)),
                 dict(offset=off(b + "sublayer_connections.1.norm.weight"), rows=1, cols=D, stats=r(5)),
@@ -645,6 +651,10 @@
                 self.measure_fwd = guard.want_measure_forward()
                 guard.eval_passes += 1
             self.off, self.wide = guard.off.copy(), guard.wide.copy()
+        self.h_planes = bool(self.use_hp and m.ffn_hidden_planes and m.weights_prep and scales[0].get("hp_2_valid")
+                             and m.dff % 512 == 0 and m.dff <= 2048 and (B * L) % 32 == 0
+                             and (not self.backward or (self.gate_mask and self.top_scales))
+                             and not (self.measure or self.measure_fwd))
 
     def prod(self, i, k, **scale_kw):
         if self.wide is not None and self.wide[i, k]:
@@ -692,22 +702,33 @@
     h2, mean2, rstd2 = K.layernorm_fwd(x2, W(b + "sublayer_connections.1.norm.weight"),
                                        W(b + "sublayer_connections.1.norm.bias"), row_scale=s_h2, planes=hplanes)
     fmask = None
+    use_b = sc is not None and not (plan.off is not None and plan.off[i, 1])
+    f1_planes = False
     if plan.use_hp and not (plan.wide is not None and plan.wide[i, 2]):
         if plan.gate_mask:
             fmask = K.gate_mask_buffer(Tn, m.dff, dev)
             m.__dict__["_gate_mask_passes"] = m.__dict__.get("_gate_mask_passes", 0) + 1
+        f1_planes = plan.h_planes and use_b and not (plan.wide is not None and plan.wide[i, 3])
+        out = None
+        if f1_planes:
+            out = K.hp_view(torch.empty(K.lib().ptamd_hp_bytes(Tn, m.dff), dtype=torch.uint8, device=dev), sc["f1_scale"], Tn, m.dff,
+                            uniform=True)
+            m.__dict__["_ffn_plane_passes"] = m.__dict__.get("_ffn_plane_passes", 0) + 1
         f1 = K.gemm_hp(K.hp_view(hplanes, s_h2, Tn, D), sc["hp_1"],
-                       torch.empty(Tn, m.dff, dtype=torch.float32, device=dev), bias=W(b + "pwff.layer1.bias"),
-                       flags=K.EPI_RELU, dropout_p=p, seed=seed, stream_id=sid + _SITE_FFN_HID, gate_mask_out=fmask)
+                       None if f1_planes else torch.empty(Tn, m.dff, dtype=torch.float32, device=dev), bias=W(b + "pwff.layer1.bias"),
+                       flags=K.EPI_RELU, dropout_p=p, seed=seed, stream_id=sid + _SITE_FFN_HID, gate_mask_out=fmask, out_planes=out)
     else:
         f1 = K.linear_fwd(h2, W(b + "pwff.layer1.weight"), W(b + "pwff.layer1.bias"), flags=K.EPI_RELU,
                           dropout_p=p, seed=seed, stream_id=sid + _SITE_FFN_HID,
                           **plan.prod(i, 2, a_scale=s_h2, b_scale=sc and sc["rs_1"]))
-    use_b = sc is not None and not (plan.off is not None and plan.off[i, 1])
-    x3 = K.linear_fwd(f1, W(b + "pwff.layer2.weight"), W(b + "pwff.layer2.bias"), residual=x2, ldr=D,
-                      dropout_p=p, seed=seed, stream_id=sid + _SITE_FFN_OUT, defer_reduce=i + 1 < m.nlayers,
-                      **plan.prod(i, 3, a_scale=sc["f1_scale"] if use_b else None, a_scale_stride=0 if use_b else 1,
-                                  b_scale=sc and sc["rs_2"]))
+    if f1_planes:
+        x3 = K.linear_fwd_hp(f1, sc["hp_2"], W(b + "pwff.layer2.bias"), residual=x2, ldr=D,
+                             dropout_p=p, seed=seed, stream_id=sid + _SITE_FFN_OUT, defer_reduce=i + 1 < m.nlayers)
+    else:
+        x3 = K.linear_fwd(f1, W(b + "pwff.layer2.weight"), W(b + "pwff.layer2.bias"), residual=x2, ldr=D,
+                          dropout_p=p, seed=seed, stream_id=sid + _SITE_FFN_OUT, defer_reduce=i + 1 < m.nlayers,
+                          **plan.prod(i, 3, a_scale=sc["f1_scale"] if use_b else None, a_scale_stride=0 if use_b else 1,
+                                      b_scale=sc and sc["rs_2"]))
     if plan.measure_fwd:
         gs = sc["guard_stats"][i]
         K.weight_scales([dict(w=t, stats=gs[j], rows_only=True) for j, t in ((0, att), (1, f1), (3, h1), (4, h2))])
@@ -780,6 +801,7 @@
             have_min = True
     uni = sc is not None and have_min
     o_att, o_f1, o_dz1, o_h1, o_h2 = (bool(v) for v in plan.off[i]) if plan.off is not None else (False,) * 5
+    f1_planes = isinstance(a.f1, K.HpOperand)
     dws.later(dy2, a.f1, G(b + "pwff.layer2.weight"), G(b + "pwff.layer2.bias"), arith=ar,
               dy_scale=sc["dy2_min"] if uni and not o_f1 else None, x_scale=sc["f1_scale"] if uni and not o_f1 else None)
     if dy2_planes is not None and have_planes and not (wide is not None and wide[i, 7]):
@@ -788,7 +810,7 @@
                         residual=a.f1 if a.fmask is None else None, ldr=a.f1.stride(0) if a.fmask is None else 0,
                         gate_mask=a.fmask, flags=K.EPI_GATE, gate_scale=1.0 / (1.0 - p))
     else:
-        dz1 = K.linear_bwd_input(dy2, W(b + "pwff.layer2.weight"), gate=a.f1, gate_dropout_p=p, gate_mask=a.fmask,
+        dz1 = K.linear_bwd_input(dy2, W(b + "pwff.layer2.weight"), gate=None if f1_planes else a.f1, gate_dropout_p=p, gate_mask=a.fmask,
                                  **plan.prod(i, 7, a_scale=s_dy2 if sc else None, b_scale=sc and sc["cs_2"]))
     if plan.measure:
         gs = sc["guard_stats"][i]
```

Measured after the change: 1.587 million residues/s, median of 6. No clear change (+0.5%).
